# Dasch0/nenbody

Hardware: AMD Instinct MI355X
Metric: body-updates/sec (N x steps/s) at N=131072, all-pairs gravity + Euler step (higher is better)
Workload: dtype f32

## Files before the change

include/nenbody.h:

```cpp
#ifndef NENBODY_H
#define NENBODY_H

#include <stddef.h>
#include <stdint.h>

#ifdef __cplusplus
extern "C" {
#endif

#define NB_ABI_VERSION 2

typedef enum nb_status {
    NB_OK = 0,
    NB_ERR_INVALID = -1,
    NB_ERR_NO_DEVICE = -2,
    NB_ERR_HIP = -3,
    NB_ERR_ALLOC = -4,
    NB_ERR_STATE = -5,
    NB_ERR_UNSUPPORTED = -6
} nb_status;

typedef enum nb_mode {
    NB_MODE_STRICT = 0,
    NB_MODE_FAST = 1
// ... 86 lines not shown

int nb_scenes_create(uint32_t scenes, uint32_t n, const nb_params *params, nb_scenes **out);
void nb_scenes_destroy(nb_scenes *ctx);
int nb_scenes_upload(nb_scenes *ctx, const float *pos_xyz, const float *vel_xyz);
int nb_scenes_step(nb_scenes *ctx, uint32_t k);
int nb_scenes_step_boids(nb_scenes *ctx, uint32_t k, const nb_boids_params *params);
int nb_scenes_download(nb_scenes *ctx, float *pos_xyz, float *vel_xyz, float *inst_16);
int nb_scenes_device_state(nb_scenes *ctx, const void **pos_rec, const void **vel_rec, const void **inst_16);
int nb_scenes_sync(nb_scenes *ctx);
uint64_t nb_scenes_steps(const nb_scenes *ctx);
const char *nb_scenes_last_error(const nb_scenes *ctx);


#include "nenbody_scenes_seen.h"


#include "nenbody_scenes_located.h"

#define NB_FRAME_MAX_DIM 4096u
int nb_camera_at(nb_ctx *ctx, const float *eye_xyz, const float *dir_xyz, const float *up_xyz, const float *cp16, float *out16);
int nb_frame(nb_ctx *ctx, const float *cam16, uint32_t width, uint32_t height, uint32_t flags, uint32_t *ids, float *depth, float *rgba,
             uint32_t *bgra8);

#define NB_FRAME_MSAA_MAX_DIM 2048u
int nb_frame_sample_offsets(float *out16);
int nb_frame_msaa(nb_ctx *ctx, const float *cam16, uint32_t width, uint32_t height, uint32_t flags, uint32_t *ids8, float *depth8,
                  float *rgba, uint32_t *bgra8);

int nb_download(nb_ctx *ctx, float *pos_xyz, float *vel_xyz, float *inst_16n);

int nb_sync(nb_ctx *ctx);

uint64_t nb_steps_done(const nb_ctx *ctx);

int nb_update_instance_nbody(float *instances_16n, size_t n_instances, float *positions_xyz, size_t n_positions,
                             float *old_positions_xyz, size_t n_old_positions, float *velocities_xyz, size_t n_velocities,
                             float *old_velocities_xyz, size_t n_old_velocities, const nb_params *params);
int nb_update_instance_boids(float *instances_16n, size_t n_instances, float *positions_xyz, size_t n_positions,
                             float *old_positions_xyz, size_t n_old_positions, float *velocities_xyz, size_t n_velocities,
                             float *old_velocities_xyz, size_t n_old_velocities, const nb_boids_params *params);
int nb_update_instance_random(float *instances_16n, size_t n_instances, float *positions_xyz, size_t n_positions,
                              float *velocities_xyz, size_t n_velocities);
int nb_update_instance_random_seeded(float *instances_16n, size_t n_instances, float *positions_xyz, size_t n_positions,
                                     float *velocities_xyz, size_t n_velocities, uint64_t seed, uint64_t step);
void nb_update_random_seed(uint64_t seed);

void nb_update_release(void);


size_t nb_scratch_bytes(const nb_params *params, uint32_t n_total, uint32_t count);

int nb_launch_step(const nb_params *params, uint32_t n_total, uint32_t first, uint32_t count, const void *pos_in,
                   void *pos_out, void *vel, void *scratch, size_t scratch_bytes, void *stream);

enum { NB_PHASE_RANGE = 0, NB_PHASE_REST = 1 };
size_t nb_scratch_bytes_phased(const nb_params *params, uint32_t n_total, uint32_t count, uint32_t j_lo, uint32_t j_hi);
int nb_launch_step_phase(const nb_params *params, uint32_t n_total, uint32_t first, uint32_t count, uint32_t j_lo, uint32_t j_hi,
                         int phase, const void *pos_in, void *pos_out, void *vel, void *scratch, size_t scratch_bytes, void *stream);

int nb_ring_partners(const nb_params *params, uint32_t n_total, uint32_t first, uint32_t count);
size_t nb_ring_scratch_bytes(const nb_params *params, uint32_t n_total, uint32_t first, uint32_t count);
int nb_launch_ring_fold(const nb_params *params, uint32_t n_total, uint32_t first, uint32_t count, const void *pos_in, void *sums,
                        void *scratch, size_t scratch_bytes, void *stream);
int nb_launch_ring_finish(const nb_params *params, uint32_t n_total, uint32_t first, uint32_t count, const void *pos_in, void *pos_out,
                          void *vel, const void *sums, const void *recv, void *stream);

enum { NB_RING_OWN = 1, NB_RING_REST = 2, NB_RING_SUMS = 3, NB_RING_OWN_READY = 4 };
int nb_ring_phased(const nb_params *params, uint32_t n_total, uint32_t first, uint32_t count);
int nb_launch_ring_fold_phase(const nb_params *params, uint32_t n_total, uint32_t first, uint32_t count, int phase, const void *pos_in,
                              void *sums, void *scratch, size_t scratch_bytes, void *stream);
int nb_launch_ring_finish_phase(const nb_params *params, uint32_t n_total, uint32_t first, uint32_t count, const void *pos_in, void *pos_out,
                                void *vel, const void *sums, const void *recv, void *scratch, size_t scratch_bytes, void *stream);

int nb_launch_boids_step(const nb_boids_params *params, uint32_t n_total, uint32_t first, uint32_t count, const void *pos_in,
                         const void *vel_in, void *pos_out, void *vel_out, void *stream);

size_t nb_boids_split_scratch_bytes(const nb_boids_params *params, uint32_t n_total, uint32_t count);
int nb_launch_boids_step_split(const nb_boids_params *params, uint32_t n_total, uint32_t first, uint32_t count, const void *pos_in,
                               const void *vel_in, void *pos_out, void *vel_out, void *scratch, size_t scratch_bytes, void *stream);

int nb_launch_instances(uint32_t count, const void *pos, const void *vel, void *inst_16n, void *stream);

int nb_launch_cameras(uint32_t count, const void *eyes, const void *dirs, const float *up_xyz, const float *cp16, void *out_16n,
                      void *stream);

int nb_launch_eyes(uint32_t n_total, uint32_t first, uint32_t count, const void *cams_16, const void *inst_16n, uint32_t width,
                   uint32_t flags, void *ids, void *depth, void *stream);

int nb_launch_seen(uint32_t count, uint32_t width, const void *ids_rows, const void *depth_rows, void *seen_count, void *seen_ids,
                   void *seen_depth, void *seen_cols, void *stream);

int nb_launch_boids_seen_step(const nb_boids_params *params, uint32_t n_total, uint32_t first, uint32_t count, const void *pos_in,
                              const void *vel_in, const void *seen_count, const void *seen_ids, uint32_t stride, void *pos_out,
                              void *vel_out, void *stream);

int nb_seen_located_launch(uint32_t count, uint32_t width, const void *ids_rows, const void *depth_rows, const void *seen_count,
                           const void *seen_ids, const void *seen_depth, const void *eyes, const void *dirs, const float *up_xyz,
                           const float *cp16, void *seen_col, void *seen_rel, void *stream);

int nb_nbody_located_step_launch(const nb_params *params, uint32_t n_total, uint32_t first, uint32_t count, const void *pos_in,
                                 const void *vel_in, const void *seen_count, const void *seen_rel, uint32_t stride, void *pos_out,
                                 void *vel_out, void *stream);

int nb_launch_eyes_colour(uint32_t n_total, uint32_t first, uint32_t count, const void *cams_16, const void *inst_16n, uint32_t width,
                          uint32_t flags, const void *skin, uint32_t tw, uint32_t th, void *ids, void *depth, void *rgba, void *bgra8,
                          void *stream);
// ... 72 lines not shown
```

include/nenbody_diag.h:

```cpp
#ifndef NENBODY_DIAG_H
#define NENBODY_DIAG_H

#include "nenbody.h"

#ifdef __cplusplus
extern "C" {
#endif

int nb_selftest_divide(const nb_params *params, uint64_t pairs, uint64_t seed, uint64_t *mismatches, float *bad_pair);

int nb_selftest_ladder(uint32_t first_significand, uint32_t count, uint64_t *mismatches, float *bad_pair);
int nb_selftest_rcp_scaling(int k_lo, int k_hi, uint64_t *violations);

int nb_selftest_matrices(uint32_t count, uint64_t seed, uint64_t *mismatches, float *bad_velocity);
int nb_selftest_libm(int fn, uint32_t first, uint64_t count, uint32_t x_bits, uint64_t *mismatches, uint32_t *first_bad);

int nb_selftest_valu_rate(int mix, double seconds, double *lane_ops_per_s, double *clock_mhz);

int nb_diag_step_clock(const nb_params *params, uint32_t n, double seconds, double *clock_mhz, double *wave_cycles,
                       double *kernel_ms);

int nb_diag_enable_env(int on);
int nb_debug_reload_env(void);

int nb_diag_rccl_solo(int on);

int nb_diag_legacy_forms(void);

int nb_diag_peers_lossy(int on);

int nb_diag_plan(const nb_params *params, uint32_t n_total, uint32_t count, char *out, size_t out_bytes);

#ifdef __cplusplus
}
#endif
#endif
```

nenbody_amd/_lib.py:

```python
from __future__ import annotations

import ctypes
import os
from ctypes import POINTER, c_char_p, c_float, c_int, c_size_t, c_uint32, c_uint64, c_void_p

_HERE = os.path.dirname(os.path.abspath(__file__))
LIB_PATH = os.environ.get("NENBODY_LIB") or os.path.join(_HERE, "lib", "libnenbody_hip.so")

NB_ABI_VERSION = 2
NB_OK = 0
NB_ERR_INVALID = -1
NB_ERR_NO_DEVICE = -2
NB_ERR_HIP = -3
NB_ERR_ALLOC = -4
NB_ERR_STATE = -5
NB_ERR_UNSUPPORTED = -6

NB_MODE_STRICT = 0
NB_MODE_FAST = 1
NB_PHASE_RANGE = 0
NB_PHASE_REST = 1
NB_RING_OWN, NB_RING_REST, NB_RING_SUMS, NB_RING_OWN_READY = 1, 2, 3, 4
NB_SCENES_MAX_BODIES = 2048
NB_EYES_NONE = 0xFFFFFFFF
NB_EYES_SEE_SELF = 1
NB_EYES_MAX_WIDTH = 4096
NB_EYES_MAX_SKIN = 2048
NB_EYES_SAMPLES = 8
NB_EYES_MSAA_MAX_WIDTH = 2048
NB_FRAME_MAX_DIM = 4096
NB_FRAME_MSAA_MAX_DIM = 2048

_STATUS_NAMES = {
    NB_ERR_INVALID: "NB_ERR_INVALID",
    NB_ERR_NO_DEVICE: "NB_ERR_NO_DEVICE",
    NB_ERR_HIP: "NB_ERR_HIP",
    NB_ERR_ALLOC: "NB_ERR_ALLOC",
    NB_ERR_STATE: "NB_ERR_STATE",
    NB_ERR_UNSUPPORTED: "NB_ERR_UNSUPPORTED",
}


class NbParams(ctypes.Structure):

    _fields_ = [("dt", c_float), ("G", c_float), ("bias", c_float), ("tile", c_uint32), ("mode", c_uint32)]

    def __repr__(self) -> str:
        return f"NbParams(dt={self.dt}, G={self.G}, bias={self.bias}, tile={self.tile}, mode={self.mode})"


class NbBoidsParams(ctypes.Structure):

    _fields_ = [("dt", c_float), ("rule_1_distance", c_float), ("rule_2_distance", c_float), ("rule_3_distance", c_float),
                ("rule_1_scale", c_float), ("rule_2_scale", c_float), ("rule_3_scale", c_float), ("tile", c_uint32)]


class NbError(RuntimeError):

    def __init__(self, status: int, message: str):
        self.status = status
        super().__init__(f"{_STATUS_NAMES.get(status, status)}: {message}")


NB_COMM_ID_BYTES = 128
GATHER_FN = ctypes.CFUNCTYPE(c_int, c_void_p, c_void_p, c_size_t, c_int, c_int, c_void_p)

RING_FN = ctypes.CFUNCTYPE(c_int, c_void_p, c_void_p, c_void_p, c_size_t, c_int, c_int, c_int, c_void_p)

PROTOTYPES = {
    "nb_abi_version": (c_int, []),
    "nb_default_params": (None, [POINTER(NbParams)]),
    "nb_device_count": (c_int, []),
    "nb_last_error": (c_char_p, [c_void_p]),
    "nb_init_state": (c_int, [c_uint64, c_uint32, c_void_p, c_void_p]),
# ... 28 lines not shown
    "nb_launch_seen": (c_int, [c_uint32, c_uint32, c_void_p, c_void_p, c_void_p, c_void_p, c_void_p, c_void_p, c_void_p]),
    "nb_step_boids_seen": (c_int, [c_void_p, c_uint32, POINTER(NbBoidsParams), c_void_p, c_void_p, c_uint32, c_uint32]),
    "nb_launch_boids_seen_step": (
        c_int, [POINTER(NbBoidsParams), c_uint32, c_uint32, c_uint32, c_void_p, c_void_p, c_void_p, c_void_p, c_uint32, c_void_p, c_void_p,
                c_void_p]),
    "nb_eyes_located": (
        c_int, [c_void_p, c_uint32, c_uint32, c_void_p, c_void_p, c_uint32, c_uint32, c_void_p, c_void_p, c_void_p, c_void_p, c_void_p,
                c_void_p]),
    "nb_seen_located_launch": (
        c_int, [c_uint32, c_uint32, c_void_p, c_void_p, c_void_p, c_void_p, c_void_p, c_void_p, c_void_p, c_void_p, c_void_p, c_void_p,
                c_void_p, c_void_p]),
    "nb_step_nbody_located": (c_int, [c_void_p, c_uint32, c_void_p, c_void_p, c_uint32, c_uint32]),
    "nb_nbody_located_step_launch": (
        c_int, [POINTER(NbParams), c_uint32, c_uint32, c_uint32, c_void_p, c_void_p, c_void_p, c_void_p, c_uint32, c_void_p, c_void_p,
                c_void_p]),
    "nb_scenes_nbody_step_launch": (c_int, [POINTER(NbParams), c_uint32, c_uint32, c_uint32, c_void_p, c_void_p, c_void_p]),
    "nb_scenes_boids_step_launch": (c_int, [POINTER(NbBoidsParams), c_uint32, c_uint32, c_uint32, c_void_p, c_void_p, c_void_p]),
    "nb_scenes_create": (c_int, [c_uint32, c_uint32, POINTER(NbParams), POINTER(c_void_p)]),
    "nb_scenes_destroy": (None, [c_void_p]),
    "nb_scenes_upload": (c_int, [c_void_p, c_void_p, c_void_p]),
    "nb_scenes_step": (c_int, [c_void_p, c_uint32]),
    "nb_scenes_step_boids": (c_int, [c_void_p, c_uint32, POINTER(NbBoidsParams)]),
    "nb_scenes_download": (c_int, [c_void_p, c_void_p, c_void_p, c_void_p]),
    "nb_scenes_device_state": (c_int, [c_void_p, POINTER(c_void_p), POINTER(c_void_p), POINTER(c_void_p)]),
    "nb_scenes_sync": (c_int, [c_void_p]),
    "nb_scenes_steps": (c_uint64, [c_void_p]),
    "nb_scenes_last_error": (c_char_p, [c_void_p]),
    "nb_srgb_decode_table": (c_int, [c_void_p]),
    "nb_srgb_encode": (c_int, [c_void_p, c_size_t, c_void_p]),
    "nb_camera_at": (c_int, [c_void_p, c_void_p, c_void_p, c_void_p, c_void_p, c_void_p]),
    "nb_frame": (c_int, [c_void_p, c_void_p, c_uint32, c_uint32, c_uint32, c_void_p, c_void_p, c_void_p, c_void_p]),
    "nb_frame_scratch_bytes": (c_size_t, [c_uint32, c_uint32]),
    "nb_launch_frame": (c_int, [c_uint32, c_void_p, c_void_p, c_uint32, c_uint32, c_uint32, c_void_p, c_uint32, c_uint32, c_void_p,
                                c_void_p, c_void_p, c_void_p, c_void_p, c_void_p]),
    "nb_frame_sample_offsets": (c_int, [c_void_p]),
    "nb_frame_msaa": (c_int, [c_void_p, c_void_p, c_uint32, c_uint32, c_uint32, c_void_p, c_void_p, c_void_p, c_void_p]),
    "nb_frame_msaa_scratch_bytes": (c_size_t, [c_uint32, c_uint32]),
    "nb_launch_frame_msaa": (c_int, [c_uint32, c_void_p, c_void_p, c_uint32, c_uint32, c_uint32, c_void_p, c_uint32, c_uint32, c_void_p,
                                     c_void_p, c_void_p, c_void_p, c_void_p, c_void_p]),
    "nb_launch_random_step": (c_int, [c_uint32, c_uint32, c_void_p, c_void_p, c_uint64, c_uint64, c_void_p]),
    "nb_update_instance_nbody": (c_int, [c_void_p, c_size_t] * 5 + [POINTER(NbParams)]),
    "nb_update_instance_boids": (c_int, [c_void_p, c_size_t] * 5 + [POINTER(NbBoidsParams)]),
    "nb_update_instance_random": (c_int, [c_void_p, c_size_t, c_void_p, c_size_t, c_void_p, c_size_t]),
    "nb_update_instance_random_seeded": (c_int, [c_void_p, c_size_t, c_void_p, c_size_t, c_void_p, c_size_t, c_uint64, c_uint64]),
    "nb_update_random_seed": (None, [c_uint64]),
    "nb_update_release": (None, []),
    "nb_sync": (c_int, [c_void_p]),
    "nb_steps_done": (c_uint64, [c_void_p]),
    "nb_scratch_bytes": (c_size_t, [POINTER(NbParams), c_uint32, c_uint32]),
    "nb_launch_step": (
        c_int,
        [POINTER(NbParams), c_uint32, c_uint32, c_uint32, c_void_p, c_void_p, c_void_p, c_void_p, c_size_t, c_void_p],
    ),
    "nb_scratch_bytes_phased": (c_size_t, [POINTER(NbParams), c_uint32, c_uint32, c_uint32, c_uint32]),
    "nb_launch_step_phase": (
        c_int,
        [POINTER(NbParams), c_uint32, c_uint32, c_uint32, c_uint32, c_uint32, c_int, c_void_p, c_void_p, c_void_p, c_void_p, c_size_t,
         c_void_p],
    ),
    "nb_ring_partners": (c_int, [POINTER(NbParams), c_uint32, c_uint32, c_uint32]),
    "nb_ring_scratch_bytes": (c_size_t, [POINTER(NbParams), c_uint32, c_uint32, c_uint32]),
    "nb_launch_ring_fold": (c_int, [POINTER(NbParams), c_uint32, c_uint32, c_uint32, c_void_p, c_void_p, c_void_p, c_size_t, c_void_p]),
    "nb_ring_phased": (c_int, [POINTER(NbParams), c_uint32, c_uint32, c_uint32]),
    "nb_launch_ring_fold_phase": (c_int, [POINTER(NbParams), c_uint32, c_uint32, c_uint32, c_int, c_void_p, c_void_p, c_void_p, c_size_t, c_void_p]),
    "nb_launch_ring_finish": (
        c_int, [POINTER(NbParams), c_uint32, c_uint32, c_uint32, c_void_p, c_void_p, c_void_p, c_void_p, c_void_p, c_void_p]),
    "nb_launch_ring_finish_phase": (
        c_int, [POINTER(NbParams), c_uint32, c_uint32, c_uint32, c_void_p, c_void_p, c_void_p, c_void_p, c_void_p, c_void_p, c_size_t, c_void_p]),
    "nb_launch_status": (c_int, [c_void_p]),
    "nb_launch_instances": (c_int, [c_uint32, c_void_p, c_void_p, c_void_p, c_void_p]),
    "nb_launch_pack": (c_int, [c_uint32, c_void_p, c_void_p, c_void_p]),
    "nb_launch_unpack": (c_int, [c_uint32, c_void_p, c_void_p, c_void_p]),
    "nb_comm_id": (c_int, [c_void_p]),
    "nb_shard_create": (c_int, [c_uint32, c_int, c_int, POINTER(NbParams), POINTER(c_void_p)]),
    "nb_shard_destroy": (None, [c_void_p]),
    "nb_shard_use_rccl": (c_int, [c_void_p, c_void_p]),
    "nb_shard_use_gather": (c_int, [c_void_p, GATHER_FN, c_void_p]),
    "nb_shard_set_overlap": (c_int, [c_void_p, c_int]),
    "nb_shard_use_ring": (c_int, [c_void_p, RING_FN, c_void_p]),
    "nb_shard_set_pairs": (c_int, [c_void_p, c_int]),
    "nb_shard_pairs_partners": (c_int, [c_void_p]),
    "nb_shard_pairs_overlapped": (c_int, [c_void_p]),
    "nb_shard_verify_exchanges": (c_int, [c_void_p, POINTER(c_int), POINTER(c_int)]),
    "nb_shard_peer_export": (c_int, [c_void_p, c_void_p]),
    "nb_shard_peer_import": (c_int, [c_void_p, c_void_p]),
    "nb_shard_use_peers": (c_int, [c_void_p, c_int]),
    "nb_peers_blob_bytes": (c_size_t, []),
    "nb_peers_create": (c_int, [c_int, c_int, POINTER(c_void_p)]),
    "nb_peers_destroy": (None, [c_void_p]),
    "nb_peers_last_error": (c_char_p, [c_void_p]),
    "nb_peers_export": (c_int, [c_void_p, POINTER(c_void_p), POINTER(c_size_t), c_int, c_void_p]),
    "nb_peers_import": (c_int, [c_void_p, c_void_p]),
    "nb_peers_probe": (c_int, [c_void_p, c_uint32]),
    "nb_peers_signal": (c_int, [c_void_p, c_int, c_void_p]),
    "nb_peers_gather": (c_int, [c_void_p, c_int, c_int, c_size_t, c_void_p]),
    "nb_peers_ring": (c_int, [c_void_p, c_int, c_int, c_void_p, c_size_t, c_int, c_void_p]),
    "nb_shard_choose_form": (c_int, [c_void_p, c_uint32, POINTER(c_int), POINTER(ctypes.c_double)]),
    "nb_shard_set_boids_split": (c_int, [c_void_p, c_int]),
    "nb_shard_range": (c_int, [c_void_p, POINTER(c_uint32), POINTER(c_uint32)]),
    "nb_shard_upload": (c_int, [c_void_p, c_void_p, c_void_p]),
    "nb_shard_step": (c_int, [c_void_p, c_uint32]),
    "nb_shard_step_boids": (c_int, [c_void_p, c_uint32, POINTER(NbBoidsParams)]),
    "nb_shard_download": (c_int, [c_void_p, c_void_p, c_void_p, c_void_p]),
    "nb_shard_sync": (c_int, [c_void_p]),
    "nb_shard_last_error": (c_char_p, [c_void_p]),
}

SCENES_SEEN_PROTOTYPES = {
    "nb_scenes_boids_seen_step_launch": (c_int, [POINTER(NbBoidsParams), c_uint32, c_uint32, c_void_p, c_void_p, c_uint32, c_void_p, c_void_p,
                                                 c_void_p, c_void_p, c_void_p]),
    "nb_scenes_seen_launch": (c_int, [c_uint32, c_uint32, c_uint32, c_uint32, c_void_p, c_void_p, c_uint32, c_void_p, c_void_p, c_void_p]),
    "nb_scenes_step_boids_seen": (c_int, [c_void_p, c_uint32, POINTER(NbBoidsParams), c_void_p, c_void_p, c_uint32]),
    "nb_scenes_eyes_seen": (c_int, [c_void_p, c_uint32, c_uint32, c_void_p, c_void_p, c_uint32, c_void_p, c_void_p]),
}

SCENES_LOCATED_PROTOTYPES = {
    "nb_scenes_nbody_located_step_launch": (c_int, [POINTER(NbParams), c_uint32, c_uint32, c_void_p, c_void_p, c_void_p, c_void_p, c_uint32,
                                                    c_void_p, c_void_p, c_void_p, c_void_p, c_void_p]),
    "nb_scenes_located_launch": (c_int, [c_uint32, c_uint32, c_uint32, c_uint32, c_void_p, c_void_p, c_void_p, c_void_p, c_void_p, c_uint32,
                                         c_void_p, c_void_p, c_void_p, c_void_p, c_void_p, c_void_p]),
    "nb_scenes_step_nbody_located": (c_int, [c_void_p, c_uint32, c_void_p, c_void_p, c_uint32]),
    "nb_scenes_eyes_located": (c_int, [c_void_p, c_uint32, c_uint32, c_void_p, c_void_p, c_uint32, c_void_p, c_void_p, c_void_p, c_void_p,
                                       c_void_p]),
}

DIAG_PROTOTYPES = {
    "nb_selftest_ladder": (c_int, [c_uint32, c_uint32, POINTER(c_uint64), c_void_p]),
    "nb_selftest_rcp_scaling": (c_int, [c_int, c_int, POINTER(c_uint64)]),
    "nb_selftest_matrices": (c_int, [c_uint32, c_uint64, POINTER(c_uint64), c_void_p]),
    "nb_selftest_libm": (c_int, [c_int, c_uint32, c_uint64, c_uint32, POINTER(c_uint64), POINTER(c_uint32)]),
    "nb_selftest_divide": (c_int, [POINTER(NbParams), c_uint64, c_uint64, POINTER(c_uint64), c_void_p]),
    "nb_selftest_valu_rate": (c_int, [c_int, ctypes.c_double, POINTER(ctypes.c_double), POINTER(ctypes.c_double)]),
    "nb_diag_step_clock": (c_int, [POINTER(NbParams), c_uint32, ctypes.c_double, POINTER(ctypes.c_double), POINTER(ctypes.c_double),
                                   POINTER(ctypes.c_double)]),
    "nb_debug_reload_env": (c_int, []),
    "nb_diag_enable_env": (c_int, [c_int]),
    "nb_diag_rccl_solo": (c_int, [c_int]),
    "nb_diag_legacy_forms": (c_int, []),
    "nb_diag_peers_lossy": (c_int, [c_int]),
    "nb_diag_plan": (c_int, [POINTER(NbParams), c_uint32, c_uint32, ctypes.c_char_p, c_size_t]),
}

_lib = None


def _preload_torch_hip_runtime() -> None:
    if os.environ.get("NENBODY_SYSTEM_HIP"):
        return
    try:
        import importlib.util

        spec = importlib.util.find_spec("torch")
        if spec is None or not spec.submodule_search_locations:
            return
        path = os.path.join(list(spec.submodule_search_locations)[0], "lib", "libamdhip64.so")
        if os.path.exists(path):
            ctypes.CDLL(path, mode=ctypes.RTLD_GLOBAL)
            rccl = os.path.join(os.path.dirname(path), "librccl.so")
            if os.path.exists(rccl):
                os.environ.setdefault("NENBODY_RCCL", rccl)
    except Exception:
        pass


_loaded = {}


def _bind(path: str) -> ctypes.CDLL:
    if path in _loaded:
        return _loaded[path]
    if not os.path.exists(path):
        raise ImportError(
            f"{path} is missing: build it with `make -C nenbody_amd/csrc` (hipcc, gfx950). "
            "nenbody_amd has no CPU fallback."
        )
    _preload_torch_hip_runtime()
    lib = ctypes.CDLL(path)
    for name, (restype, argtypes) in list(PROTOTYPES.items()) + list(SCENES_SEEN_PROTOTYPES.items()) + list(SCENES_LOCATED_PROTOTYPES.items()) \
            + list(DIAG_PROTOTYPES.items()):
        fn = getattr(lib, name)
        fn.restype = restype
        fn.argtypes = argtypes
    got = lib.nb_abi_version()
    if got != NB_ABI_VERSION:
        raise ImportError(f"{os.path.basename(path)} ABI {got} != binding ABI {NB_ABI_VERSION}")
    _loaded[path] = lib
    return lib


def load() -> ctypes.CDLL:
    global _lib
    if _lib is None:
        _lib = _bind(LIB_PATH)
# ... 92 lines not shown
```

nenbody_amd/csrc/nb_api.hip:

```cpp
#include <hip/hip_runtime.h>
#include <dlfcn.h>

#include <cmath>
#include <cstdlib>
#include <algorithm>
#include <atomic>
#include <chrono>
#include <cstring>
#include <mutex>
#include <new>
#include <string>
#include <thread>
#include <vector>

#include "../../include/nenbody.h"
#include "../../include/nenbody_diag.h"
#include "nb_kernels.h"
#include "nb_plan.h"
#include "nb_eyes.h"
#include "nb_frame.h"
#include "nb_seen.h"
#include "nb_located.h"
#include "nb_scenes.h"
#define NB_SRGB_TABLE static const
// ... 17 lines not shown
using nbp::valid_tile;

Knob read_knob(const char *name)
{
    Knob k;
    const char *s = std::getenv(name);
    if (s && *s) {
        k.set = true;
        k.v = (uint32_t)std::strtoul(s, nullptr, 10);
    }
    return k;
}

std::atomic<const DebugOverrides *> g_overrides{nullptr};
std::atomic<bool> g_env_enabled{false};
std::atomic<bool> g_rccl_solo{false};
std::mutex g_overrides_mu;

const DebugOverrides *parse_overrides(uint32_t generation)
{
    DebugOverrides *d = new DebugOverrides();
    d->generation = generation;
    d->roctx = read_knob("NB_ROCTX");
    if (!g_env_enabled.load(std::memory_order_relaxed)) return d;
    for (const nbp::KnobName &k : nbp::kKnobNames) d->*k.knob = read_knob(k.name);
    return d;
}

const DebugOverrides &overrides()
{
    const DebugOverrides *d = g_overrides.load(std::memory_order_acquire);
    if (d) return *d;
    std::lock_guard<std::mutex> lock(g_overrides_mu);
    d = g_overrides.load(std::memory_order_acquire);
    if (!d) {
        d = parse_overrides(1);
        g_overrides.store(d, std::memory_order_release);
    }
    return *d;
}

int make_plan(const nb_params &p, uint32_t n_total, uint32_t count, Plan *out, std::string *err)
{
    return nbp::make_plan(p, n_total, count, overrides(), out, err);
}

struct KernelSizes {
    size_t planes_bytes(uint32_t n) const { return nbk::strict_bc_scratch_bytes(n); }
    uint32_t pairs_chunk(uint32_t n, uint32_t chunk) const { return nbk::fast_pairs_chunk(n, chunk); }
    uint32_t pairs_rows(uint32_t n, uint32_t w, uint32_t np) const { return nbk::fast_pairs_rows(n, w, np); }
    size_t pairs_scratch_floats(uint32_t n, uint32_t w, uint32_t np, uint32_t chunk) const { return nbk::fast_pairs_scratch_floats(n, w, np, chunk); }
};
size_t plan_scratch_bytes(const Plan &pl, uint32_t count) { return nbp::plan_scratch_bytes(pl, count, KernelSizes{}); }

struct PlanKey {
    nb_params p;
    uint32_t shape[4];
    uint32_t generation;
};
PlanKey plan_key(const nb_params &p, uint32_t s0, uint32_t s1, uint32_t s2 = 0, uint32_t s3 = 0)
{
    PlanKey k;
    std::memset(&k, 0, sizeof(k));
    k.p = p;
    k.shape[0] = s0;
    k.shape[1] = s1;
    k.shape[2] = s2;
    k.shape[3] = s3;
    k.generation = overrides().generation;
    return k;
}
template <typename Key, typename Value, int N>
class PlanCache {
    struct Entry {
        bool valid = false;
        Key key;
        Value value;
    };
    Entry entries_[N];
    int next_ = 0;

public:
    template <typename Make>
    int get(const Key &key, const Value **out, Make make)
    {
        for (const Entry &e : entries_)
            if (e.valid && std::memcmp(&e.key, &key, sizeof(Key)) == 0) {
                *out = &e.value;
                return NB_OK;
            }
        Value v;
        int rc = make(&v);
        if (rc != NB_OK) return rc;
        Entry &e = entries_[next_];
        next_ = (next_ + 1) % N;
        e.valid = true;
        e.key = key;
        e.value = v;
        *out = &e.value;
        return NB_OK;
    }
};

int cached_plan(const nb_params &p, uint32_t n_total, uint32_t count, const Plan **out, std::string *err)
{
    thread_local PlanCache<PlanKey, Plan, 4> cache;
// ... 91 lines not shown
}

struct StatusWord {
    uint32_t *w = nullptr;
    bool dirty = false;
};

int status_word_for_launch(StatusWord *sw, std::string *err)
{
    if (!sw->w) {
        hipError_t e = hipMalloc((void **)&sw->w, 64);
        if (e == hipSuccess) e = hipMemset(sw->w, 0, 64);
        if (e != hipSuccess) {
            *err = std::string("nb: allocating the status word failed: ") + hipGetErrorString(e);
            return e == hipErrorOutOfMemory ? NB_ERR_ALLOC : NB_ERR_HIP;
        }
    }
    sw->dirty = true;
    return NB_OK;
}

int check_status(StatusWord *sw, std::string *err)
{
    if (!sw->dirty) return NB_OK;
    sw->dirty = false;
    return check_status_word(sw->w, err);
}

nbk::StepArgs step_args(const nb_params &p, const Plan &pl, uint32_t n_total, uint32_t first, uint32_t count, const void *pos_in,
                        void *pos_out, void *vel, void *partial = nullptr)
{
    nbk::StepArgs a{};
    a.pos_in = (const float4 *)pos_in;
    a.pos_out = (float4 *)pos_out;
    a.vel = (float4 *)vel;
    a.partial = (float4 *)partial;
    a.n_total = n_total;
    a.first = first;
    a.count = count;
    a.dt = p.dt;
    a.G = p.G;
    a.bias = p.bias;
    a.j_count = n_total;
    a.hole_lo = 0xffffffffu;
    nbp::plan_step_args(pl, &a);
    return a;
}

struct Launchers {
    const nbk::StepArgs &a;
    void *scratch;
    uint32_t *status;
    hipStream_t s;
    hipError_t strict(uint32_t tile, uint32_t unroll, uint32_t lanes) const { return nbk::launch_strict(a, tile, unroll, lanes, s); }
    hipError_t strict_pc(uint32_t producers) const { return nbk::launch_strict_pc(a, producers, s); }
    hipError_t strict_bc() const { return nbk::launch_strict_bc(a, scratch, status, s); }
    hipError_t strict_sl(uint32_t shape) const { return nbk::launch_strict_sl(a, shape, scratch, s); }
    hipError_t fast(uint32_t tile, uint32_t ib, uint32_t groups, uint32_t slices) const { return nbk::launch_fast(a, tile, ib, groups, slices, s); }
    hipError_t fast_wave(uint32_t tile, uint32_t ib, uint32_t waves, uint32_t slices) const { return nbk::launch_fast_wave(a, tile, ib, waves, slices, s); }
    hipError_t fast_sl(uint32_t ib, uint32_t slices) const { return nbk::launch_fast_sl(a, ib, slices, scratch, s); }
    hipError_t fast_pairs(uint32_t w, uint32_t np, uint32_t chunk) const { return nbk::launch_fast_pairs(a, w, np, chunk, scratch, s); }
};
hipError_t launch_planned(const Plan &pl, const nbk::StepArgs &a, void *scratch, uint32_t *status, hipStream_t stream)
{
    return nbp::visit_launch(pl, Launchers{a, scratch, status, stream});
}

int launch_status(hipError_t e, const char *what, std::string *err)
{
    if (e == hipSuccess) return NB_OK;
    *err = std::string(what) + hipGetErrorString(e);
    return NB_ERR_HIP;
}

int launch_step_planned(const nb_params &p, const Plan &pl, uint32_t n_total, uint32_t first, uint32_t count,
                        const void *pos_in, void *pos_out, void *vel, void *scratch, hipStream_t stream, std::string *err,
                        StatusWord *sw = nullptr)
{
    const nbk::StepArgs a = step_args(p, pl, n_total, first, count, pos_in, pos_out, vel, scratch);
    uint32_t *status = nullptr;
    if (nbp::form_info(pl.form).status_word) {
        int rc = sw ? status_word_for_launch(sw, err) : device_status_word(&status, err);
        if (rc != NB_OK) return rc;
        if (sw) status = sw->w;
    }
    hipError_t e = launch_planned(pl, a, scratch, status, stream);
    if (e == hipErrorNotSupported) {
        *err = "nb: this launch shape is one of the legacy forms (NB_STRICT_PC / NB_STRICT_LANES / NB_STRICT_UNROLL / NB_STRICT_SL=2,3 / "
               "NB_FAST_WAVES / NB_FAST_GROUPS / NB_FAST_PAIRS_W): this library was built without them (make -C nenbody_amd/csrc legacy "
               "builds libnenbody_hip_legacy.so, which holds every form)";
        return NB_ERR_UNSUPPORTED;
    }
    return launch_status(e, "nb: kernel launch failed: ", err);
}

int check_device(std::string *err)
{
    static std::atomic<bool> seen{false};
    if (seen.load(std::memory_order_relaxed)) return NB_OK;
    int n = 0;
    hipError_t e = hipGetDeviceCount(&n);
    if (e != hipSuccess || n <= 0) {
        (void)hipGetLastError();
        *err = std::string("nb: no HIP device available (") + (e == hipSuccess ? "0 devices" : hipGetErrorString(e)) +
               "); this library has no CPU path";
        return NB_ERR_NO_DEVICE;
    }
    seen.store(true, std::memory_order_relaxed);
    return NB_OK;
}

float sqrt_threshold(float r)
{
    if (!(r > 0.0f)) return -1.0f;
    uint32_t lo = 0u, hi = 0x7f7fffffu;
    auto below = [&](uint32_t b) {
        float x;
        std::memcpy(&x, &b, 4);
        return std::sqrt(x) < r;
    };
    if (!below(lo)) return -1.0f;
    if (below(hi)) {
        float x;
        std::memcpy(&x, &hi, 4);
        return x;
    }
    while (hi - lo > 1u) {
        const uint32_t mid = lo + (hi - lo) / 2u;
        if (below(mid))
            lo = mid;
        else
            hi = mid;
    }
    float x;
    std::memcpy(&x, &lo, 4);
    return x;
}

float rule3_always_bound(float t3)
// ... 196 lines not shown
        p = nullptr;
        cells = 0;
    }
    hipError_t reserve(size_t want)
    {
        if (want <= cells) return hipSuccess;
        release();
        const hipError_t e = hipMalloc((void **)&p, want * sizeof(T));
        if (e == hipSuccess)
            cells = want;
        else
            p = nullptr;
        return e;
    }
    void swap(DeviceBuffer &other)
    {
        std::swap(p, other.p);
        std::swap(cells, other.cells);
    }
};

struct nb_ctx {
    uint32_t n = 0;
    nb_params p{};
    Plan plan{};
    hipStream_t stream = nullptr;
    DeviceBuffer<float4> pos[2];
    DeviceBuffer<float4> vel;
    DeviceBuffer<float4> vel_alt;
    DeviceBuffer<float> stage;
    DeviceBuffer<float4> inst;
    DeviceBuffer<float4> cams;
    DeviceBuffer<uint32_t> eye_ids;
    DeviceBuffer<float> eye_depth;
    DeviceBuffer<float4> eye_rgba;
    DeviceBuffer<uint32_t> eye_bgra;
    DeviceBuffer<uint32_t> seen_count;
    DeviceBuffer<uint32_t> seen_ids;
    DeviceBuffer<float> seen_depth;
    DeviceBuffer<uint32_t> seen_cols;
    DeviceBuffer<uint32_t> loc_col;
    DeviceBuffer<float4> loc_rel;
    DeviceBuffer<float> skin;
    uint32_t skin_w = 0, skin_h = 0;
    DeviceBuffer<uint64_t> frame_keys;
    DeviceBuffer<float4> frame_cam;
    DeviceBuffer<float> xfer;
    float *hxfer = nullptr;
    float *hxfer_dev = nullptr;
    DeviceBuffer<uint32_t> done_counter;
    uint32_t done_seq = 0, polled_calls = 0;
    uint32_t poll_holdoff = 0, poll_backoff = 0;
    DeviceBuffer<char> scratch;
    StatusWord status;
    int cur = 0;
    bool uploaded = false;
    uint64_t steps = 0;
    std::string err;
    ~nb_ctx()
    {
        if (hxfer) (void)hipHostFree(hxfer);
        if (status.w) (void)hipFree(status.w);
    }
};

#define NB_HIP(ctx, call)                                                                          \
    do {                                                                                           \
        hipError_t e_ = (call);                                                                    \
        if (e_ != hipSuccess) {                                                                    \
            (ctx)->err = std::string("nb: " #call " failed: ") + hipGetErrorString(e_);            \
            return (e_ == hipErrorOutOfMemory) ? NB_ERR_ALLOC : NB_ERR_HIP;                        \
        }                                                                                          \
    } while (0)

static const char kCallUpload[] = " (call nb_upload first)";
static const char kCallScenesUpload[] = " (call nb_scenes_upload first)";
template <typename Ctx>
static int ctx_check(Ctx *ctx, const char *fn, const char *state_hint = nullptr)
{
    if (!ctx) {
        g_tls_error = std::string(fn) + ": ctx is null";
        return NB_ERR_INVALID;
    }
    if (state_hint && !ctx->uploaded) {
        ctx->err = std::string(fn) + ": no state uploaded" + state_hint;
        return NB_ERR_STATE;
    }
    return NB_OK;
}

static hipError_t launch_matrices(uint32_t n, const float4 *pos, const float4 *vel, DeviceBuffer<float4> *inst, hipStream_t stream)
{
    const hipError_t e = inst->reserve((size_t)n * 4);
    if (e != hipSuccess) return e;
    return nbk::launch_instances(n, pos, vel, inst->p, stream, overrides().inst_device_libm.on() ? 1u : 0u);
}

static void step_done(nb_ctx *c, bool wrote_vel_alt)
{
    c->cur ^= 1;
    if (wrote_vel_alt) c->vel.swap(c->vel_alt);
    c->steps++;
}

NB_EXPORT int nb_abi_version(void) { return NB_ABI_VERSION; }

NB_EXPORT void nb_default_params(nb_params *p)
{
    if (!p) return;
    p->dt = 0.1f;
    p->G = 0.001f;
    p->bias = 0.0000001f;
    p->tile = 0;
    p->mode = NB_MODE_STRICT;
}

NB_EXPORT int nb_device_count(void)
{
    int n = 0;
    hipError_t e = hipGetDeviceCount(&n);
    if (e != hipSuccess) {
        (void)hipGetLastError();
        g_tls_error = std::string("nb: hipGetDeviceCount failed: ") + hipGetErrorString(e);
        return NB_ERR_NO_DEVICE;
    }
    return n;
}

NB_EXPORT const char *nb_last_error(const nb_ctx *ctx) { return ctx ? ctx->err.c_str() : g_tls_error.c_str(); }

NB_EXPORT int nb_init_state(uint64_t seed, uint32_t n, float *pos_xyz, float *vel_xyz)
{
    if (!pos_xyz || !vel_xyz) {
        g_tls_error = "nb_init_state: null array";
        return NB_ERR_INVALID;
    }
    uint64_t s = seed;
    for (uint32_t i = 0; i < n; ++i) {
        vel_xyz[3 * (size_t)i + 0] = uniform_f32(s, -0.0f, 0.1f);
        vel_xyz[3 * (size_t)i + 1] = uniform_f32(s, -0.0f, 0.1f);
        vel_xyz[3 * (size_t)i + 2] = 0.0f;
    }
    for (uint32_t i = 0; i < n; ++i) {
        pos_xyz[3 * (size_t)i + 0] = uniform_f32(s, -100.0f, 100.0f);
        pos_xyz[3 * (size_t)i + 1] = uniform_f32(s, -100.0f, 100.0f);
        pos_xyz[3 * (size_t)i + 2] = 0.0f;
    }
    return NB_OK;
}

NB_EXPORT void nb_destroy(nb_ctx *ctx)
{
// ... 49 lines not shown
    }
    if (polled) {
        d.counter = c->done_counter.p;
        d.word = (uint32_t *)(c->hxfer_dev + 22 * (size_t)c->n + kDoneWordAt);
        d.seq = ++c->done_seq ? c->done_seq : ++c->done_seq;
    }
    return d;
}

static inline void cpu_relax()
{
#if defined(__x86_64__) || defined(__i386__)
    __builtin_ia32_pause();
#elif defined(__aarch64__)
    __asm__ __volatile__("yield");
#else
    std::this_thread::yield();
#endif
}

static int wait_export(nb_ctx *c, const nbk::ExportDone &d)
{
    if (d.word) {
        const volatile uint32_t *const w = (const volatile uint32_t *)(c->hxfer + 22 * (size_t)c->n + kDoneWordAt);
        const auto kPollBudget = std::chrono::microseconds(overrides().dropin_poll_budget_us.or_else(2000u));
        const auto t0 = std::chrono::steady_clock::now();
        for (uint32_t spins = 1;; ++spins) {
            if (*w == d.seq) {
                std::atomic_thread_fence(std::memory_order_acquire);
                c->poll_backoff = 0;
                if ((++c->polled_calls & 1023u) == 0u) NB_HIP(c, hipStreamSynchronize(c->stream));
                return NB_OK;
            }
            if ((spins & 255u) == 0u && std::chrono::steady_clock::now() - t0 > kPollBudget) break;
            cpu_relax();
        }
        c->poll_backoff = c->poll_backoff ? std::min(c->poll_backoff * 2u, 4096u) : 64u;
        c->poll_holdoff = c->poll_backoff;
        NB_HIP(c, hipStreamSynchronize(c->stream));
        if (*w != d.seq) NB_HIP(c, hipMemsetAsync(c->done_counter.p, 0, sizeof(uint32_t), c->stream));
        return NB_OK;
    }
    NB_HIP(c, hipStreamSynchronize(c->stream));
    return NB_OK;
}

static int create_impl(nb_ctx *c)
{
    NB_HIP(c, hipStreamCreateWithFlags(&c->stream, hipStreamNonBlocking));
    NB_HIP(c, c->pos[0].reserve(c->n));
    NB_HIP(c, c->pos[1].reserve(c->n));
    NB_HIP(c, c->vel.reserve(c->n));
    NB_HIP(c, c->stage.reserve((size_t)c->n * 3));
    NB_HIP(c, c->scratch.reserve(plan_scratch_bytes(c->plan, c->n)));
    return NB_OK;
}

NB_EXPORT int nb_create(uint32_t n, uint32_t n_devices, const nb_params *params, nb_ctx **out)
{
    if (!out) {
        g_tls_error = "nb_create: out is null";
        return NB_ERR_INVALID;
    }
    *out = nullptr;
    if (n_devices != 1) {
        g_tls_error =
            "nb_create: n_devices must be 1 (one process drives one GPU; shard with nb_launch_step and an all-gather)";
        return NB_ERR_UNSUPPORTED;
    }
    const nb_params p = params_or_default(params);
    Plan plan;
    int rc = make_plan(p, n, n, &plan, &g_tls_error);
    if (rc != NB_OK) return rc;
    rc = check_device(&g_tls_error);
    if (rc != NB_OK) return rc;
    nb_ctx *c = new (std::nothrow) nb_ctx();
    if (!c) {
        g_tls_error = "nb_create: out of host memory";
        return NB_ERR_ALLOC;
    }
    c->n = n;
    c->p = p;
    c->plan = plan;
    rc = create_impl(c);
    if (rc != NB_OK) {
        g_tls_error = c->err;
        nb_destroy(c);
        return rc;
    }
    *out = c;
    return NB_OK;
}


static int small_import(nb_ctx *c, const float *pos_xyz, const float *vel_xyz)
{
    const size_t n = c->n, bytes = n * 3 * sizeof(float);
    std::memcpy(c->hxfer, pos_xyz, bytes);
    std::memcpy(c->hxfer + 3 * n, vel_xyz, bytes);
    float *src = c->hxfer_dev;
    if (!small_set_zero_copy(c->n)) {
        NB_HIP(c, hipMemcpyAsync(c->xfer.p, c->hxfer, 2 * bytes, hipMemcpyHostToDevice, c->stream));
        src = c->xfer.p;
    }
    NB_HIP(c, nbk::launch_import(c->n, src, src + 3 * n, c->pos[0].p, c->vel.p, c->stream));
    return NB_OK;
}

static int small_export(nb_ctx *c, bool inst, bool pos, bool vel, bool *with_status)
{
    const size_t n = c->n;
    const bool zero_copy = small_set_zero_copy(c->n);
    float *const dst = zero_copy ? c->hxfer_dev : c->xfer.p;
    const bool ws = *with_status = c->status.dirty && c->status.w;
    const nbk::ExportDone done = export_done(c, small_set_poll(c->n));
    NB_HIP(c, nbk::launch_export(c->n, c->pos[c->cur].p, c->vel.p, inst ? (float4 *)dst : nullptr, pos ? dst + 16 * n : nullptr,
                                 vel ? dst + 19 * n : nullptr, ws ? c->status.w : nullptr, ws ? (uint32_t *)(dst + 22 * n) : nullptr,
                                 c->stream, overrides().inst_device_libm.on() ? 1u : 0u, done));
    if (!zero_copy) {
        const size_t lo = inst ? 0 : (pos ? 16 * n : 19 * n), hi = ws ? 22 * n + 1 : vel ? 22 * n : (pos ? 19 * n : 16 * n);
        NB_HIP(c, hipMemcpyAsync(c->hxfer + lo, c->xfer.p + lo, (hi - lo) * sizeof(float), hipMemcpyDeviceToHost, c->stream));
    }
    return wait_export(c, done);
}

NB_EXPORT int nb_upload(nb_ctx *ctx, const float *pos_xyz, const float *vel_xyz)
{
    int rc = ctx_check(ctx, "nb_upload");
    if (rc != NB_OK) return rc;
    if (!pos_xyz || !vel_xyz) {
        ctx->err = "nb_upload: null array";
        return NB_ERR_INVALID;
    }
    const size_t bytes = (size_t)ctx->n * 3 * sizeof(float);
    ctx->cur = 0;
    if (ctx->n <= kRoundtripMax) {
        rc = ensure_xfer(ctx);
        if (rc != NB_OK) return rc;
        NB_HIP(ctx, hipStreamSynchronize(ctx->stream));
        rc = small_import(ctx, pos_xyz, vel_xyz);
        if (rc != NB_OK) return rc;
        NB_HIP(ctx, hipStreamSynchronize(ctx->stream));
        ctx->uploaded = true;
        ctx->steps = 0;
        return NB_OK;
    }
    NB_HIP(ctx, hipMemcpyAsync(ctx->stage.p, pos_xyz, bytes, hipMemcpyHostToDevice, ctx->stream));
    NB_HIP(ctx, nbk::launch_pack(ctx->n, ctx->stage.p, ctx->pos[0].p, ctx->stream));
    NB_HIP(ctx, hipStreamSynchronize(ctx->stream));
    NB_HIP(ctx, hipMemcpyAsync(ctx->stage.p, vel_xyz, bytes, hipMemcpyHostToDevice, ctx->stream));
    NB_HIP(ctx, nbk::launch_pack(ctx->n, ctx->stage.p, ctx->vel.p, ctx->stream));
    NB_HIP(ctx, hipStreamSynchronize(ctx->stream));
    ctx->uploaded = true;
    ctx->steps = 0;
    return NB_OK;
}

NB_EXPORT int nb_step(nb_ctx *ctx, uint32_t k)
{
    int rc = ctx_check(ctx, "nb_step", kCallUpload);
    if (rc != NB_OK) return rc;
    RoctxRange range("nb_step");
    for (uint32_t s = 0; s < k; ++s) {
        rc = launch_step_planned(ctx->p, ctx->plan, ctx->n, 0, ctx->n, ctx->pos[ctx->cur].p, ctx->pos[ctx->cur ^ 1].p, ctx->vel.p,
                                 ctx->scratch.p, ctx->stream, &ctx->err, &ctx->status);
        if (rc != NB_OK) return rc;
        step_done(ctx, false);
    }
    return NB_OK;
}

NB_EXPORT void nb_boids_default_params(nb_boids_params *p)
{
    if (!p) return;
    p->dt = 0.04f;
    p->rule_1_distance = 1000.0f;
    p->rule_2_distance = 5.0f;
    p->rule_3_distance = 500.0f;
    p->rule_1_scale = 0.02f;
    p->rule_2_scale = 0.05f;
    p->rule_3_scale = 0.5f;
    p->tile = 0;
}

NB_EXPORT int nb_step_boids(nb_ctx *ctx, uint32_t k, const nb_boids_params *params)
{
    int rc = ctx_check(ctx, "nb_step_boids", kCallUpload);
    if (rc != NB_OK) return rc;
    const nb_boids_params p = boids_params_or_default(params);
    nbk::BoidsArgs a;
    uint32_t tile = 0;
    rc = make_boids_args(p, ctx->n, 0, ctx->n, &a, &tile, &ctx->err);
    if (rc != NB_OK) return rc;
    NB_HIP(ctx, ctx->vel_alt.reserve(ctx->n));
    RoctxRange range("nb_step_boids");
    for (uint32_t s = 0; s < k; ++s) {
        a.pos_in = ctx->pos[ctx->cur].p;
        a.pos_out = ctx->pos[ctx->cur ^ 1].p;
        a.vel_in = ctx->vel.p;
        a.vel_out = ctx->vel_alt.p;
        NB_HIP(ctx, nbk::launch_boids(a, tile, boids_form(a.count), ctx->stream));
        step_done(ctx, true);
    }
    return NB_OK;
}

NB_EXPORT int nb_step_random(nb_ctx *ctx, uint32_t k, uint64_t seed)
{
    const int rc = ctx_check(ctx, "nb_step_random", kCallUpload);
    if (rc != NB_OK) return rc;
    for (uint32_t s = 0; s < k; ++s) {
        NB_HIP(ctx, nbk::launch_random(0, ctx->n, ctx->pos[ctx->cur].p, ctx->vel.p, seed, ctx->steps, ctx->stream));
        ctx->steps++;
    }
    return NB_OK;
}

NB_EXPORT int nb_device_state(nb_ctx *ctx, const void **pos_rec, const void **vel_rec, const void **inst_16n)
{
    const int rc = ctx_check(ctx, "nb_device_state", "");
    if (rc != NB_OK) return rc;
    if (inst_16n) {
        NB_HIP(ctx, launch_matrices(ctx->n, ctx->pos[ctx->cur].p, ctx->vel.p, &ctx->inst, ctx->stream));
        *inst_16n = ctx->inst.p;
    }
    if (pos_rec) *pos_rec = ctx->pos[ctx->cur].p;
    if (vel_rec) *vel_rec = ctx->vel.p;
    return NB_OK;
}

NB_EXPORT int nb_camera_constant(float vertical_fov_deg, float aspect_ratio, float near_plane, float far_plane, float *cp16)
{
    if (!cp16) {
        g_tls_error = "nb_camera_constant: cp16 is null";
        return NB_ERR_INVALID;
    }
    const float pi = (float)3.14159265358979323846;
    const float fovy = vertical_fov_deg * (float)(3.14159265358979323846 / 180.0);
    if (!(fovy > 0.0f) || !(fovy < pi) || !(aspect_ratio != 0.0f) || !(near_plane > 0.0f) || !(far_plane > 0.0f) || !(far_plane != near_plane)) {
        g_tls_error = "nb_camera_constant: cgmath::perspective asserts 0 < fovy < 180 degrees, aspect != 0, near > 0, far > 0, far != near";
        return NB_ERR_INVALID;
    }
    const float f = 1.0f / std::tan(fovy / 2.0f);
    float proj[16] = {0.0f};
    proj[0] = f / aspect_ratio;
    proj[5] = f;
    proj[10] = (far_plane + near_plane) / (near_plane - far_plane);
    proj[11] = -1.0f;
    proj[14] = ((2.0f * far_plane) * near_plane) / (near_plane - far_plane);
    const float corr[16] = {1.0f, 0.0f, 0.0f, 0.0f, 0.0f, 1.0f, 0.0f, 0.0f, 0.0f, 0.0f, 0.5f, 0.0f, 0.0f, 0.0f, 0.5f, 1.0f};
    for (int col = 0; col < 4; ++col)
        for (int row = 0; row < 4; ++row) {
            const float t0 = corr[row] * proj[4 * col], t1 = corr[4 + row] * proj[4 * col + 1];
            const float t2 = corr[8 + row] * proj[4 * col + 2], t3 = corr[12 + row] * proj[4 * col + 3];
            cp16[4 * col + row] = ((t0 + t1) + t2) + t3;
        }
    return NB_OK;
}

NB_EXPORT int nb_cameras(nb_ctx *ctx, const float *up_xyz, const float *cp16, float *out_16n)
{
    int rc = ctx_check(ctx, "nb_cameras");
    if (rc != NB_OK) return rc;
    if (!up_xyz || !cp16 || !out_16n) {
// ... 359 lines not shown
NB_EXPORT uint64_t nb_steps_done(const nb_ctx *ctx) { return ctx ? ctx->steps : 0; }

NB_EXPORT int nb_download(nb_ctx *ctx, float *pos_xyz, float *vel_xyz, float *inst_16n)
{
    int rc = ctx_check(ctx, "nb_download", "");
    if (rc != NB_OK) return rc;
    const size_t bytes = (size_t)ctx->n * 3 * sizeof(float);
    if (ctx->n <= kRoundtripMax && (pos_xyz || vel_xyz || inst_16n)) {
        rc = ensure_xfer(ctx);
        if (rc != NB_OK) return rc;
        const size_t n = ctx->n;
        bool with_status = false;
        rc = small_export(ctx, inst_16n != nullptr, pos_xyz != nullptr, vel_xyz != nullptr, &with_status);
        if (rc != NB_OK) return rc;
        if (inst_16n) std::memcpy(inst_16n, ctx->hxfer, n * 16 * sizeof(float));
        if (pos_xyz) std::memcpy(pos_xyz, ctx->hxfer + 16 * n, bytes);
        if (vel_xyz) std::memcpy(vel_xyz, ctx->hxfer + 19 * n, bytes);
        return status_from_tail(ctx, with_status);
    }
    if (pos_xyz) {
        NB_HIP(ctx, nbk::launch_unpack(ctx->n, ctx->pos[ctx->cur].p, ctx->stage.p, ctx->stream));
        NB_HIP(ctx, hipMemcpyAsync(pos_xyz, ctx->stage.p, bytes, hipMemcpyDeviceToHost, ctx->stream));
        NB_HIP(ctx, hipStreamSynchronize(ctx->stream));
    }
    if (vel_xyz) {
        NB_HIP(ctx, nbk::launch_unpack(ctx->n, ctx->vel.p, ctx->stage.p, ctx->stream));
        NB_HIP(ctx, hipMemcpyAsync(vel_xyz, ctx->stage.p, bytes, hipMemcpyDeviceToHost, ctx->stream));
        NB_HIP(ctx, hipStreamSynchronize(ctx->stream));
    }
    if (inst_16n) {
        NB_HIP(ctx, launch_matrices(ctx->n, ctx->pos[ctx->cur].p, ctx->vel.p, &ctx->inst, ctx->stream));
        NB_HIP(ctx, hipMemcpyAsync(inst_16n, ctx->inst.p, (size_t)ctx->n * 16 * sizeof(float), hipMemcpyDeviceToHost,
                                   ctx->stream));
        NB_HIP(ctx, hipStreamSynchronize(ctx->stream));
    }
    if (!pos_xyz && !vel_xyz && !inst_16n) NB_HIP(ctx, hipStreamSynchronize(ctx->stream));
    return check_status(&ctx->status, &ctx->err);
}

#include "nb_dropin.inc"

#include "nb_selftest.inc"


NB_EXPORT size_t nb_scratch_bytes(const nb_params *params, uint32_t n_total, uint32_t count)
{
    const nb_params p = params_or_default(params);
    Plan pl;
    std::string err;
    if (make_plan(p, n_total, count, &pl, &err) != NB_OK) return 0;
    return plan_scratch_bytes(pl, count);
}

NB_EXPORT int nb_launch_step(const nb_params *params, uint32_t n_total, uint32_t first, uint32_t count, const void *pos_in,
                             void *pos_out, void *vel, void *scratch, size_t scratch_bytes, void *stream)
{
    const nb_params p = params_or_default(params);
    if (!pos_in || !pos_out || !vel || pos_in == pos_out) {
        g_tls_error = "nb_launch_step: pos_in, pos_out, vel must be non-null and pos_out must not alias pos_in";
        return NB_ERR_INVALID;
    }
    if ((uint64_t)first + (uint64_t)count > (uint64_t)n_total) {
        g_tls_error = "nb_launch_step: [first, first+count) exceeds n_total";
        return NB_ERR_INVALID;
    }
    const Plan *pl = nullptr;
    int rc = cached_plan(p, n_total, count, &pl, &g_tls_error);
    if (rc != NB_OK) return rc;
    const size_t need = plan_scratch_bytes(*pl, count);
    if (need && (!scratch || scratch_bytes < need)) {
        g_tls_error = "nb_launch_step: scratch smaller than nb_scratch_bytes()";
        return NB_ERR_INVALID;
    }
    rc = device_for_launch(pos_in, stream, SelectDevice::kForNullStream);
    if (rc != NB_OK) return rc;
    return launch_step_planned(p, *pl, n_total, first, count, pos_in, pos_out, vel, scratch, (hipStream_t)stream, &g_tls_error);
}

NB_EXPORT int nb_launch_status(void *stream)
{
    int rc = check_device(&g_tls_error);
    if (rc != NB_OK) return rc;
    int cur = -1, restore = -1;
    if (stream) {
        hipDevice_t sdev = -1;
        if (hipStreamGetDevice((hipStream_t)stream, &sdev) == hipSuccess && hipGetDevice(&cur) == hipSuccess && sdev >= 0 && sdev != cur) {
            if (hipSetDevice(sdev) == hipSuccess) restore = cur;
        } else {
            (void)hipGetLastError();
        }
    }
    hipError_t e = hipStreamSynchronize((hipStream_t)stream);
    if (e != hipSuccess) {
        g_tls_error = std::string("nb_launch_status: hipStreamSynchronize failed: ") + hipGetErrorString(e);
        rc = NB_ERR_HIP;
    } else {
        rc = check_device_status(&g_tls_error);
    }
    if (restore >= 0) (void)hipSetDevice(restore);
    return rc;
}

namespace {
int make_phase_plan(const nb_params &p, uint32_t n_total, uint32_t count, uint32_t j_lo, uint32_t j_hi, PhasePlan *out, std::string *err)
{
    return nbp::make_phase_plan(p, n_total, count, j_lo, j_hi, overrides(), out, err);
}
size_t phase_scratch_bytes(const PhasePlan &pp, uint32_t count) { return nbp::phase_scratch_bytes(pp, count, KernelSizes{}); }

int cached_phase_plan(const nb_params &p, uint32_t n_total, uint32_t count, uint32_t j_lo, uint32_t j_hi, const PhasePlan **out,
                      std::string *err)
{
    thread_local PlanCache<PlanKey, PhasePlan, 2> cache;
    return cache.get(plan_key(p, n_total, count, j_lo, j_hi), out,
                     [&](PhasePlan *pp) { return make_phase_plan(p, n_total, count, j_lo, j_hi, pp, err); });
}
}

NB_EXPORT size_t nb_scratch_bytes_phased(const nb_params *params, uint32_t n_total, uint32_t count, uint32_t j_lo, uint32_t j_hi)
{
    const nb_params p = params_or_default(params);
    PhasePlan pp;
    std::string err;
    if (make_phase_plan(p, n_total, count, j_lo, j_hi, &pp, &err) != NB_OK) return 0;
    return phase_scratch_bytes(pp, count);
}

namespace {
int launch_phase_planned(const nb_params &p, const PhasePlan &pp, uint32_t n_total, uint32_t first, uint32_t count, uint32_t j_lo,
// ... 23 lines not shown
        a.hole_len = pp.len[0];
        e = fold(1, false, 0, 0);
        if (e == hipSuccess) e = nbk::launch_integrate_partials(a, pp.slices[0] + pp.slices[1], stream);
    }
    return launch_status(e, "nb: kernel launch failed (step phase): ", err);
}
}

NB_EXPORT int nb_launch_step_phase(const nb_params *params, uint32_t n_total, uint32_t first, uint32_t count, uint32_t j_lo,
                                   uint32_t j_hi, int phase, const void *pos_in, void *pos_out, void *vel, void *scratch,
                                   size_t scratch_bytes, void *stream)
{
    const nb_params p = params_or_default(params);
    if (!pos_in || !pos_out || !vel || pos_in == pos_out || !scratch || (phase != NB_PHASE_RANGE && phase != NB_PHASE_REST)) {
        g_tls_error = "nb_launch_step_phase: pos_in, pos_out, vel, scratch must be non-null, pos_out must not alias pos_in, phase is "
                      "NB_PHASE_RANGE or NB_PHASE_REST";
        return NB_ERR_INVALID;
    }
    if ((uint64_t)first + (uint64_t)count > (uint64_t)n_total) {
        g_tls_error = "nb_launch_step_phase: [first, first+count) exceeds n_total";
        return NB_ERR_INVALID;
    }
    const PhasePlan *ppp = nullptr;
    int rc = cached_phase_plan(p, n_total, count, j_lo, j_hi, &ppp, &g_tls_error);
    if (rc != NB_OK) return rc;
    const PhasePlan &pp = *ppp;
    if (scratch_bytes < phase_scratch_bytes(pp, count)) {
        g_tls_error = "nb_launch_step_phase: scratch smaller than nb_scratch_bytes_phased()";
        return NB_ERR_INVALID;
    }
    rc = device_for_launch(pos_in, stream, SelectDevice::kForNullStream);
    if (rc != NB_OK) return rc;
    return launch_phase_planned(p, pp, n_total, first, count, j_lo, phase, pos_in, pos_out, vel, scratch, (hipStream_t)stream, &g_tls_error);
}

#include "nb_ring_api.inc"


NB_EXPORT int nb_diag_legacy_forms(void)
{
#ifdef NB_LEGACY_FORMS
    return 1;
#else
    return 0;
#endif
}

NB_EXPORT int nb_diag_rccl_solo(int on)
{
    g_rccl_solo.store(on != 0, std::memory_order_relaxed);
    return NB_OK;
}

NB_EXPORT int nb_diag_plan(const nb_params *params, uint32_t n_total, uint32_t count, char *out, size_t out_bytes)
{
    if (!out || out_bytes == 0) {
        g_tls_error = "nb_diag_plan: out is null";
        return NB_ERR_INVALID;
    }
    const nb_params p = params_or_default(params);
    Plan pl;
    int rc = make_plan(p, n_total, count, &pl, &g_tls_error);
    if (rc != NB_OK) return rc;
    const std::string k = nbp::plan_kernels(pl, KernelSizes{});
    if (k.size() + 1 > out_bytes) {
        g_tls_error = "nb_diag_plan: out too small";
        return NB_ERR_INVALID;
    }
    std::memcpy(out, k.c_str(), k.size() + 1);
    return NB_OK;
}

namespace {
int reread_overrides(bool enable)
{
    std::lock_guard<std::mutex> lock(g_overrides_mu);
    g_env_enabled.store(enable, std::memory_order_relaxed);
    const DebugOverrides *old = g_overrides.load(std::memory_order_acquire);
    g_overrides.store(parse_overrides(old ? old->generation + 1u : 1u), std::memory_order_release);
    return NB_OK;
}
}
NB_EXPORT int nb_diag_enable_env(int on) { return reread_overrides(on != 0); }
NB_EXPORT int nb_debug_reload_env(void) { return reread_overrides(true); }

NB_EXPORT int nb_launch_boids_step(const nb_boids_params *params, uint32_t n_total, uint32_t first, uint32_t count,
                                   const void *pos_in, const void *vel_in, void *pos_out, void *vel_out, void *stream)
{
    const nb_boids_params p = boids_params_or_default(params);
    if (!pos_in || !vel_in || !pos_out || !vel_out || pos_in == pos_out || vel_in == vel_out) {
        g_tls_error = "nb_launch_boids_step: buffers must be non-null and the outputs must not alias the inputs";
        return NB_ERR_INVALID;
    }
    nbk::BoidsArgs a;
    uint32_t tile = 0;
    int rc = make_boids_args(p, n_total, first, count, &a, &tile, &g_tls_error);
    if (rc != NB_OK) return rc;
    rc = device_for_launch(pos_in, stream, SelectDevice::kAlways);
    if (rc != NB_OK) return rc;
    a.pos_in = (const float4 *)pos_in;
    a.vel_in = (const float4 *)vel_in;
    a.pos_out = (float4 *)pos_out;
    a.vel_out = (float4 *)vel_out;
    return launch_status(nbk::launch_boids(a, tile, boids_form(a.count), (hipStream_t)stream), "nb: boids kernel launch failed: ", &g_tls_error);
}

// ... 224 lines not shown
```

nenbody_amd/csrc/nb_kernels.h:

```cpp
#pragma once
#include <hip/hip_runtime.h>
#include <stdint.h>

namespace nbk {

struct StepArgs {
    const float4 *pos_in;
    float4 *pos_out;
    float4 *vel;
    float4 *partial;
    uint32_t n_total, first, count;
    float dt, G, bias;
    uint32_t lo_bits, hi_bits;
    uint32_t force_ieee;
    uint32_t force_3d;
    uint32_t j_chunk;
    uint32_t no_packed;
    uint32_t spin_budget;
    uint32_t bc_prio;
    uint32_t j_count, j_base, hole_lo, hole_len;
    uint32_t partial_row0;
    uint32_t always_partial;
    unsigned long long *stamps;
};

struct BoidsMaskK {
    float k1, tk1;
    float k2, tk2;
    float k3, tk3;
};

struct BoidsArgs {
    const float4 *pos_in;
    const float4 *vel_in;
    float4 *pos_out;
    float4 *vel_out;
    uint32_t n_total, first, count;
    float dt;
    float r1;
    float t2, t3;
    float s1, s2, s3;
    uint32_t force_flags;
    uint32_t vlim_bits;
    float4 *partial;
    uint32_t j_chunk;
    float4 *vtot;
    uint32_t *gflags;
    uint32_t mk_valid;
    BoidsMaskK mk;
};
hipError_t launch_boids(const BoidsArgs &a, uint32_t tile, uint32_t form, hipStream_t s);
hipError_t launch_boids_split(const BoidsArgs &a, uint32_t tile, uint32_t slices, hipStream_t s);

hipError_t launch_strict(const StepArgs &a, uint32_t tile, uint32_t unroll, uint32_t lanes, hipStream_t s);
hipError_t launch_strict_jp(const StepArgs &a, uint32_t tile, uint32_t unroll, uint32_t lanes, hipStream_t s);
hipError_t launch_strict_pc(const StepArgs &a, uint32_t producers, hipStream_t s);
hipError_t launch_strict_bc(const StepArgs &a, void *scratch, uint32_t *status, hipStream_t s);
size_t strict_bc_scratch_bytes(uint32_t n_total);
struct PlaneScratch {
    uint32_t *flags;
    float *px, *py, *pz;
    char *behind;
    uint32_t npad;
};
PlaneScratch plane_scratch(void *scratch, uint32_t n_total);
hipError_t launch_strict_sl(const StepArgs &a, uint32_t shape, void *scratch, hipStream_t s);
hipError_t launch_strict_sl_kernel(const StepArgs &a, uint32_t shape, const uint32_t *flags, uint32_t generation, const float *px,
                                   const float *py, const float *pz, hipStream_t s);
hipError_t launch_fast(const StepArgs &a, uint32_t tile, uint32_t ib, uint32_t groups, uint32_t slices, hipStream_t s);
hipError_t launch_fast_wave(const StepArgs &a, uint32_t tile, uint32_t ib, uint32_t waves, uint32_t slices, hipStream_t s);
hipError_t launch_fast_sl(const StepArgs &a, uint32_t ib, uint32_t slices, void *scratch, hipStream_t s);
hipError_t launch_fast_sl_phase(const StepArgs &a, uint32_t ib, uint32_t slices, bool range, uint32_t r0, uint32_t r1, void *scratch,
                                hipStream_t s);
hipError_t launch_fast_sl_kernel(const StepArgs &a, uint32_t ib, uint32_t slices, const uint32_t *flags, uint32_t generation,
                                 const float *px, const float *py, const float *pz, hipStream_t s);
hipError_t launch_fast_pairs(const StepArgs &a, uint32_t w, uint32_t np, uint32_t chunk, void *scratch, hipStream_t s);
hipError_t launch_fast_pairs_kernels(const StepArgs &a, uint32_t w, uint32_t np, uint32_t chunk, const uint32_t *flags, uint32_t generation,
                                     const float *px, const float *py, const float *pz, float *scratch, hipStream_t s);
uint32_t fast_pairs_rows(uint32_t n_total, uint32_t w, uint32_t np);
size_t fast_pairs_scratch_floats(uint32_t n_total, uint32_t w, uint32_t np, uint32_t chunk);
uint32_t fast_pairs_chunk(uint32_t n_total, uint32_t chunk);
uint32_t ring_partners(uint32_t n_total, uint32_t first, uint32_t count, uint32_t np);
size_t ring_scratch_floats(uint32_t n_total, uint32_t first, uint32_t count, uint32_t np, uint32_t ga, uint32_t wpb, uint32_t c4_own = 0, uint32_t c4_rest = 0,
                           uint32_t cap = 0);
bool ring_phased(uint32_t n_total, uint32_t first, uint32_t count, uint32_t np, uint32_t ga, uint32_t wpb, uint32_t *c4_own = nullptr, uint32_t *c4_rest = nullptr,
                 uint32_t *cap = nullptr);
hipError_t launch_fast_ring_phase(const StepArgs &a, uint32_t np, uint32_t ga, uint32_t wpb, uint32_t c4_own, uint32_t c4_rest, uint32_t cap, uint32_t what,
                                  void *scratch, float4 *sums, hipStream_t s);
hipError_t launch_ring_phase_kernels(const StepArgs &a, uint32_t np, uint32_t ga, uint32_t wpb, uint32_t c4_own, uint32_t c4_rest, uint32_t cap, uint32_t what,
                                     const uint32_t *flags, const float *px, const float *py, const float *pz, float *scratch, float4 *sums,
                                     hipStream_t s);
hipError_t launch_fast_ring(const StepArgs &a, uint32_t np, uint32_t ga, uint32_t wpb, void *scratch, float4 *sums, hipStream_t s);
hipError_t launch_fast_ring_kernels(const StepArgs &a, uint32_t np, uint32_t ga, uint32_t wpb, const uint32_t *flags, uint32_t generation,
                                    const float *px, const float *py, const float *pz, float *scratch, float4 *sums, hipStream_t s);
hipError_t launch_ring_finish(const StepArgs &a, const float4 *sums, const float4 *recv, uint32_t partners, hipStream_t s);
hipError_t launch_fast_ring_finish_phase(const StepArgs &a, uint32_t np, uint32_t ga, uint32_t wpb, uint32_t c4_own, uint32_t c4_rest, uint32_t cap, void *scratch,
                                         const float4 *sums, const float4 *recv, hipStream_t s);
hipError_t launch_ring_finish_phase_kernel(const StepArgs &a, uint32_t np, uint32_t ga, uint32_t wpb, uint32_t c4_own, uint32_t c4_rest, uint32_t cap,
                                           uint32_t *flags, float *px, float *py, float *pz, float *scratch, const float4 *sums, const float4 *recv,
                                           uint32_t gen_next, hipStream_t s);
hipError_t launch_integrate_partials(const StepArgs &a, uint32_t rows, hipStream_t s);
hipError_t launch_instances(uint32_t count, const float4 *pos, const float4 *vel, float4 *inst, hipStream_t s, uint32_t device_libm = 0);
hipError_t launch_cameras(uint32_t count, const float4 *eyes, const float4 *dirs, const float *up3, const float *cp16, float4 *out,
                          hipStream_t s);
hipError_t launch_random(uint32_t first, uint32_t count, float4 *pos, float4 *vel, uint64_t seed, uint64_t step, hipStream_t s);
hipError_t launch_divide_selftest(uint32_t blocks, uint64_t seed, uint32_t per_thread, int d_lo, int d_hi, int n_lo, int n_hi,
                                  unsigned long long *mismatches, float *first_bad, bool single_correction, hipStream_t s);
hipError_t launch_ladder_exhaustive(uint32_t first_md, uint32_t count_md, bool control, unsigned long long *mismatches, float *first_bad,
                                    hipStream_t s);
hipError_t launch_rcp_scaling(int k_lo, int k_hi, unsigned long long *violations, hipStream_t s);
hipError_t launch_libm_selftest(int fn, uint32_t first, uint32_t count, uint32_t other, uint32_t *out, hipStream_t s);
hipError_t launch_valu_stream(int mix, uint32_t blocks, uint32_t trips, float *sink, unsigned long long *stamps, hipStream_t s);
hipError_t launch_unstage(uint32_t slot, uint32_t world, const float4 *stage, float4 *pos, float4 *vel, hipStream_t s);
hipError_t launch_exchange_pattern(float4 *dst, uint32_t count, float rank, float salt, bool fill_nan, hipStream_t s);
hipError_t launch_exchange_check(const float4 *src, uint32_t count, float rank, float salt, uint32_t *mismatches, hipStream_t s);
constexpr int kPeerMax = 16;
struct PullArgs {
    const float4 *src[kPeerMax];
    float4 *dst[kPeerMax];
    uint32_t copies, records;
};
hipError_t launch_peer_pull(const PullArgs &a, hipStream_t s);
hipError_t launch_pack(uint32_t count, const float *xyz, float4 *rec, hipStream_t s);
hipError_t launch_unpack(uint32_t count, const float4 *rec, float *xyz, hipStream_t s);
hipError_t launch_import(uint32_t count, const float *pos_xyz, const float *vel_xyz, float4 *pos_rec, float4 *vel_rec, hipStream_t s);
struct ExportDone {
    uint32_t *counter = nullptr;
    uint32_t *word = nullptr;
    uint32_t seq = 0;
// ... 6 lines not shown
```

nenbody_amd/csrc/nb_launch.inc:

```

static inline uint32_t ceil_div(uint32_t a, uint32_t b) { return (a + b - 1u) / b; }

template <int TJ, int U, int S>
static hipError_t launch_strict_t(const StepArgs &a, hipStream_t s)
{
    hipLaunchKernelGGL((step_strict_kernel<TJ, U, S>), dim3(ceil_div(a.count, kBlock / S)), dim3(kBlock), 0, s, a);
    return hipGetLastError();
}

#define NBK_CASE(T, U_, S_) \
    if (tile == T && unroll == U_ && lanes == S_) return launch_strict_t<T, U_, S_>(a, s)

#ifdef NBK_NOSLP_TU
hipError_t launch_strict_jp(const StepArgs &a, uint32_t tile, uint32_t unroll, uint32_t lanes, hipStream_t s)
{
    NBK_CASE(256, 2, 16);
    NBK_CASE(1024, 2, 16);
#ifdef NB_LEGACY_FORMS
    NBK_CASE(256, 4, 2);
    NBK_CASE(256, 2, 2);
    NBK_CASE(256, 4, 4);
    NBK_CASE(256, 2, 4);
    NBK_CASE(256, 4, 8);
    NBK_CASE(256, 2, 8);
    NBK_CASE(256, 4, 16);
    NBK_CASE(1024, 4, 2);
    NBK_CASE(1024, 4, 4);
    NBK_CASE(1024, 4, 8);
    NBK_CASE(1024, 2, 8);
#endif
    return hipErrorNotSupported;
}

#else
hipError_t launch_strict_pc(const StepArgs &a, uint32_t producers, hipStream_t s)
{
#ifdef NB_LEGACY_FORMS
    if (producers == 8)
        hipLaunchKernelGGL(step_strict_pc_kernel<8>, dim3(ceil_div(a.count, 64)), dim3(PcShape<8>::kThreads), 0, s, a);
    else if (producers == 14)
        hipLaunchKernelGGL(step_strict_pc_kernel<14>, dim3(ceil_div(a.count, 64)), dim3(PcShape<14>::kThreads), 0, s, a);
    else
        return hipErrorInvalidValue;
    return hipGetLastError();
#else
    return hipErrorNotSupported;
#endif
}

constexpr size_t kPlaneSlackBytes = 64;
size_t strict_bc_scratch_bytes(uint32_t n_total) { return (size_t)kBcFlagsBytes + 3u * (size_t)bc_padded(n_total) * sizeof(float) + kPlaneSlackBytes; }

PlaneScratch plane_scratch(void *scratch, uint32_t n_total)
{
    PlaneScratch v;
    v.npad = bc_padded(n_total);
    v.flags = (uint32_t *)scratch;
    v.px = (float *)((char *)scratch + kBcFlagsBytes);
    v.py = v.px + v.npad;
    v.pz = v.py + v.npad;
    v.behind = (char *)scratch + strict_bc_scratch_bytes(n_total);
    return v;
}

static std::atomic<uint32_t> g_bc_generation{0};
static uint32_t next_plane_generation()
{
    uint32_t gen = g_bc_generation.fetch_add(1u, std::memory_order_relaxed) + 1u;
    if (gen == 0u) gen = g_bc_generation.fetch_add(1u, std::memory_order_relaxed) + 1u;
    return gen;
}

static void enqueue_planes(const StepArgs &a, const PlaneScratch &v, uint32_t lo_bits, uint32_t hi_bits, uint32_t gen, hipStream_t s)
{
    hipLaunchKernelGGL(planes_kernel, dim3(ceil_div(v.npad, kBlock)), dim3(kBlock), 0, s, a.n_total, v.npad, a.pos_in, v.px, v.py, v.pz,
                       v.flags, lo_bits, hi_bits, 0u, gen);
}
constexpr uint32_t kFastPlaneLoBits = 0u, kFastPlaneHiBits = 0x4d7fffffu;
static hipError_t launch_fast_planes(const StepArgs &a, const PlaneScratch &v, uint32_t gen, hipStream_t s)
{
    enqueue_planes(a, v, kFastPlaneLoBits, kFastPlaneHiBits, gen, s);
    return hipGetLastError();
}

hipError_t launch_strict_bc(const StepArgs &a, void *scratch, uint32_t *status, hipStream_t s)
{
    const PlaneScratch v = plane_scratch(scratch, a.n_total);
    const uint32_t gen = next_plane_generation();
    enqueue_planes(a, v, a.lo_bits, a.hi_bits, gen, s);
    hipLaunchKernelGGL(step_strict_bc_kernel, dim3(ceil_div(a.count, 64)), dim3(kBcThreads), 0, s, a, (const uint32_t *)v.flags, gen,
                       (const float *)v.px, (const float *)v.py, (const float *)v.pz, status);
    return hipGetLastError();
}

hipError_t launch_strict_sl(const StepArgs &a, uint32_t shape, void *scratch, hipStream_t s)
{
    const PlaneScratch v = plane_scratch(scratch, a.n_total);
    const uint32_t gen = next_plane_generation();
    enqueue_planes(a, v, a.lo_bits, a.hi_bits, gen, s);
    hipError_t e = hipGetLastError();
    if (e != hipSuccess) return e;
    return launch_strict_sl_kernel(a, shape, v.flags, gen, v.px, v.py, v.pz, s);
}

hipError_t launch_strict(const StepArgs &a, uint32_t tile, uint32_t unroll, uint32_t lanes, hipStream_t s)
{
    if (lanes > 1) return launch_strict_jp(a, tile, unroll, lanes, s);
    NBK_CASE(256, 8, 1);
    NBK_CASE(512, 8, 1);
    NBK_CASE(1024, 8, 1);
#ifdef NB_LEGACY_FORMS
    NBK_CASE(256, 4, 1);
    NBK_CASE(512, 4, 1);
    NBK_CASE(1024, 4, 1);
    NBK_CASE(1024, 16, 1);
#endif
    return hipErrorNotSupported;
}
#endif
#undef NBK_CASE

#ifndef NBK_NOSLP_TU
hipError_t launch_integrate_partials(const StepArgs &a, uint32_t rows, hipStream_t s)
{
    hipLaunchKernelGGL(integrate_partials_kernel, dim3(ceil_div(a.count, kBlock)), dim3(kBlock), 0, s, a, rows);
    return hipGetLastError();
}

template <int TJ, int IB, int G>
static hipError_t launch_fast_t(const StepArgs &a, uint32_t slices, hipStream_t s)
{
    hipLaunchKernelGGL((step_fast_kernel<TJ, IB, G>), dim3(ceil_div(a.count, kBlock * IB), slices), dim3(kBlock * G), 0, s, a);
    hipError_t e = hipGetLastError();
    if (e != hipSuccess || slices == 1 || a.always_partial) return e;
    return launch_integrate_partials(a, slices, s);
}

hipError_t launch_fast(const StepArgs &a, uint32_t tile, uint32_t ib, uint32_t groups, uint32_t slices, hipStream_t s)
{
#ifndef NB_LEGACY_FORMS
    return hipErrorNotSupported;
#else
#define NBK_CASE(T, I, G_) \
    if (tile == T && ib == I && groups == G_) return launch_fast_t<T, I, G_>(a, slices, s)
    NBK_CASE(256, 1, 1);
    NBK_CASE(256, 2, 1);
    NBK_CASE(256, 4, 1);
    NBK_CASE(512, 1, 1);
    NBK_CASE(512, 2, 1);
    NBK_CASE(512, 4, 1);
    NBK_CASE(1024, 1, 1);
    NBK_CASE(1024, 2, 1);
    NBK_CASE(1024, 4, 1);
    NBK_CASE(256, 1, 2);
    NBK_CASE(256, 2, 2);
    NBK_CASE(256, 4, 2);
    NBK_CASE(512, 1, 2);
    NBK_CASE(512, 2, 2);
    NBK_CASE(512, 4, 2);
    NBK_CASE(256, 1, 4);
    NBK_CASE(256, 2, 4);
    NBK_CASE(256, 4, 4);
    NBK_CASE(512, 1, 4);
    NBK_CASE(512, 2, 4);
    NBK_CASE(512, 4, 4);
#undef NBK_CASE
    return hipErrorInvalidValue;
#endif
}

template <int TJ, int IB, int W>
static hipError_t launch_fast_wave_t(const StepArgs &a, uint32_t slices, hipStream_t s)
{
    hipLaunchKernelGGL((step_fast_wave_kernel<TJ, IB, W>), dim3(ceil_div(a.count, 64 * IB), slices), dim3(64 * W), 0, s, a);
    hipError_t e = hipGetLastError();
    if (e != hipSuccess || slices == 1 || a.always_partial) return e;
    return launch_integrate_partials(a, slices, s);
}

hipError_t launch_fast_wave(const StepArgs &a, uint32_t tile, uint32_t ib, uint32_t waves, uint32_t slices, hipStream_t s)
{
#define NBK_CASE(T, I, W_) \
    if (tile == T && ib == I && waves == W_) return launch_fast_wave_t<T, I, W_>(a, slices, s)
    NBK_CASE(256, 1, 8);
    NBK_CASE(256, 2, 8);
    NBK_CASE(256, 4, 8);
    NBK_CASE(512, 2, 8);
    NBK_CASE(512, 4, 8);
#ifdef NB_LEGACY_FORMS
    NBK_CASE(256, 1, 1);
    NBK_CASE(256, 1, 4);
    NBK_CASE(256, 1, 16);
    NBK_CASE(256, 2, 1);
    NBK_CASE(256, 2, 4);
    NBK_CASE(256, 2, 16);
    NBK_CASE(256, 4, 1);
    NBK_CASE(256, 4, 4);
    NBK_CASE(256, 4, 16);
    NBK_CASE(512, 2, 4);
    NBK_CASE(512, 2, 16);
    NBK_CASE(512, 4, 4);
    NBK_CASE(512, 4, 16);
#endif
#undef NBK_CASE
    return hipErrorNotSupported;
}

hipError_t launch_fast_sl(const StepArgs &a_in, uint32_t ib, uint32_t slices, void *scratch, hipStream_t s)
{
    StepArgs a = a_in;
    const PlaneScratch v = plane_scratch(scratch, a.n_total);
    a.partial = (float4 *)v.behind;
    const uint32_t gen = next_plane_generation();
    hipError_t e = launch_fast_planes(a, v, gen, s);
    if (e != hipSuccess) return e;
    e = launch_fast_sl_kernel(a, ib, slices, v.flags, gen, v.px, v.py, v.pz, s);
    if (e != hipSuccess || slices == 1 || a.always_partial) return e;
    return launch_integrate_partials(a, slices, s);
}

hipError_t launch_fast_sl_phase(const StepArgs &a_in, uint32_t ib, uint32_t slices, bool range, uint32_t r0, uint32_t r1, void *scratch,
                                hipStream_t s)
{
    StepArgs a = a_in;
    const PlaneScratch v = plane_scratch(scratch, a.n_total);
    a.partial = (float4 *)v.behind;
    const uint32_t gen = next_plane_generation();
    hipError_t e;
    if (range) {
        hipLaunchKernelGGL(planes_range_kernel, dim3(ceil_div(a.n_total, kBlock)), dim3(kBlock), 0, s, a.n_total, a.pos_in, v.px, v.py, v.pz, v.flags,
                           r0, r1, a.first, a.first + a.count, kFastPlaneLoBits, kFastPlaneHiBits, 0u, gen);
        e = hipGetLastError();
    } else {
        e = launch_fast_planes(a, v, gen, s);
    }
    if (e != hipSuccess) return e;
    return launch_fast_sl_kernel(a, ib, slices, v.flags, gen, v.px, v.py, v.pz, s);
}

hipError_t launch_fast_pairs(const StepArgs &a, uint32_t w, uint32_t np, uint32_t chunk, void *scratch, hipStream_t s)
{
    const PlaneScratch v = plane_scratch(scratch, a.n_total);
    const uint32_t gen = next_plane_generation();
    hipError_t e = launch_fast_planes(a, v, gen, s);
    if (e != hipSuccess) return e;
    return launch_fast_pairs_kernels(a, w, np, chunk, v.flags, gen, v.px, v.py, v.pz, (float *)v.behind, s);
}

hipError_t launch_fast_ring(const StepArgs &a, uint32_t np, uint32_t ga, uint32_t wpb, void *scratch, float4 *sums, hipStream_t s)
{
    const PlaneScratch v = plane_scratch(scratch, a.n_total);
    const uint32_t gen = next_plane_generation();
    hipError_t e = launch_fast_planes(a, v, gen, s);
    if (e != hipSuccess) return e;
    return launch_fast_ring_kernels(a, np, ga, wpb, v.flags, gen, v.px, v.py, v.pz, (float *)v.behind, sums, s);
}

hipError_t launch_fast_ring_phase(const StepArgs &a, uint32_t np, uint32_t ga, uint32_t wpb, uint32_t c4_own, uint32_t c4_rest, uint32_t cap, uint32_t what,
                                  void *scratch, float4 *sums, hipStream_t s)
{
    const PlaneScratch v = plane_scratch(scratch, a.n_total);
    if (what == 1u || what == 2u) {
        const uint32_t gen = next_plane_generation();
        const bool own = what == 1u;
        const uint32_t r0 = own ? a.first : 0u, r1 = own ? a.first + a.count : a.n_total;
        hipLaunchKernelGGL(ring_planes_kernel, dim3(ceil_div(r1 - r0, kBlock)), dim3(kBlock), 0, s, a.n_total, a.pos_in, v.px, v.py, v.pz,
                           v.flags + (own ? kRingFlagsNext : kRingFlagsRest), r0, r1, gen, own ? (const uint32_t *)nullptr : v.flags + kRingFlagsNext,
                           own ? (uint32_t *)nullptr : v.flags + kRingFlagsOwn);
        hipError_t e = hipGetLastError();
        if (e != hipSuccess) return e;
    }
    return launch_ring_phase_kernels(a, np, ga, wpb, c4_own, c4_rest, cap, what, v.flags, v.px, v.py, v.pz, (float *)v.behind, sums, s);
}

hipError_t launch_fast_ring_finish_phase(const StepArgs &a, uint32_t np, uint32_t ga, uint32_t wpb, uint32_t c4_own, uint32_t c4_rest, uint32_t cap, void *scratch,
                                         const float4 *sums, const float4 *recv, hipStream_t s)
{
    const PlaneScratch v = plane_scratch(scratch, a.n_total);
    return launch_ring_finish_phase_kernel(a, np, ga, wpb, c4_own, c4_rest, cap, v.flags, v.px, v.py, v.pz, (float *)v.behind, sums, recv,
                                           next_plane_generation(), s);
}

hipError_t launch_instances(uint32_t count, const float4 *pos, const float4 *vel, float4 *inst, hipStream_t s, uint32_t device_libm)
{
    hipLaunchKernelGGL(instances_kernel, dim3(ceil_div(count, kBlock)), dim3(kBlock), 0, s, count, pos, vel, inst, device_libm);
    return hipGetLastError();
}

hipError_t launch_pack(uint32_t count, const float *xyz, float4 *rec, hipStream_t s)
{
    hipLaunchKernelGGL(pack_kernel, dim3(ceil_div(count, kBlock)), dim3(kBlock), 0, s, count, xyz, rec);
    return hipGetLastError();
}

hipError_t launch_unpack(uint32_t count, const float4 *rec, float *xyz, hipStream_t s)
{
    hipLaunchKernelGGL(unpack_kernel, dim3(ceil_div(count, kBlock)), dim3(kBlock), 0, s, count, rec, xyz);
    return hipGetLastError();
}
// ... 18 lines not shown
```

nenbody_amd/csrc/nb_nbody_bc.inc:

```

#if defined(NB_EXP_BC_WAVES)
constexpr int kBcWaves = NB_EXP_BC_WAVES;
#else
constexpr int kBcWaves = 12;
#endif
constexpr int kBcThreads = kBcWaves * 64;
constexpr int kBcBlock = 64;
constexpr int kBcBlock3d = 32;
constexpr uint32_t kBcSpinBudget = 1u << 24;
static_assert(kBcBlock == kPlanePad, "planes are padded to whole blocks");

__global__ __launch_bounds__(kBlock) void planes_kernel(uint32_t n, uint32_t npad, const float4 *__restrict__ pos, float *__restrict__ px,
                                                        float *__restrict__ py, float *__restrict__ pz, uint32_t *__restrict__ flags,
                                                        uint32_t lo_bits, uint32_t hi_bits, uint32_t force, uint32_t generation)
{
    const uint32_t j = blockIdx.x * (uint32_t)kBlock + threadIdx.x;
    uint32_t f = force;
    if (j < npad) {
        const float4 r = j < n ? pos[j] : make_float4(0.f, 0.f, 0.f, 0.f);
        px[j] = r.x;
        py[j] = r.y;
        pz[j] = r.z;
        const uint32_t span = hi_bits - lo_bits;
        f |= coord_oor(r.x, lo_bits, span) | coord_oor(r.y, lo_bits, span) | coord_oor(r.z, lo_bits, span) | nonzero_bits(r.z);
    }
    f = wave_or(f);
    if ((threadIdx.x & 63) == 0) {
        if (f & kFlagIeee) flags[kBcFlagWordIeee] = generation;
        if (f & kFlagNonPlanar) flags[kBcFlagWordNonPlanar] = generation;
    }
}

__global__ __launch_bounds__(kBlock) void planes_range_kernel(uint32_t n, const float4 *__restrict__ pos, float *__restrict__ px,
                                                              float *__restrict__ py, float *__restrict__ pz, uint32_t *__restrict__ flags,
                                                              uint32_t r0, uint32_t r1, uint32_t f0, uint32_t f1, uint32_t lo_bits,
                                                              uint32_t hi_bits, uint32_t force, uint32_t generation)
{
    const uint32_t j = blockIdx.x * (uint32_t)kBlock + threadIdx.x;
    uint32_t f = force;
    if (j < n && ((j >= r0 && j < r1) || (j >= f0 && j < f1))) {
        const float4 r = pos[j];
        px[j] = r.x;
        py[j] = r.y;
        pz[j] = r.z;
        const uint32_t span = hi_bits - lo_bits;
        f |= coord_oor(r.x, lo_bits, span) | coord_oor(r.y, lo_bits, span) | coord_oor(r.z, lo_bits, span) | nonzero_bits(r.z);
    }
    f = wave_or(f);
    if ((threadIdx.x & 63) == 0) {
        if (f & kFlagIeee) flags[kBcFlagWordIeee] = generation;
        if (f & kFlagNonPlanar) flags[kBcFlagWordNonPlanar] = generation;
    }
}

__global__ __launch_bounds__(kBlock) void ring_planes_kernel(uint32_t n, const float4 *__restrict__ pos, float *__restrict__ px,
                                                             float *__restrict__ py, float *__restrict__ pz, uint32_t *__restrict__ flags,
                                                             uint32_t r0, uint32_t r1, uint32_t generation, const uint32_t *move_from,
                                                             uint32_t *move_to)
{
    if (move_from && blockIdx.x == 0 && threadIdx.x < 3u) move_to[threadIdx.x] = move_from[threadIdx.x];
    const uint32_t j = r0 + blockIdx.x * (uint32_t)kBlock + threadIdx.x;
    uint32_t f = 0u;
    if (j < r1 && j < n) {
        const float4 r = pos[j];
        px[j] = r.x;
        py[j] = r.y;
        pz[j] = r.z;
        constexpr uint32_t span = 0x4d7fffffu;
        f |= coord_oor(r.x, 0u, span) | coord_oor(r.y, 0u, span) | coord_oor(r.z, 0u, span) | nonzero_bits(r.z);
    }
    f = wave_or(f);
    if ((threadIdx.x & 63) == 0) {
        if (f & kFlagIeee) flags[kBcFlagWordIeee] = generation;
        if (f & kFlagNonPlanar) flags[kBcFlagWordNonPlanar] = generation;
        if (blockIdx.x == 0 && threadIdx.x == 0) flags[kRingGenWord] = generation;
// ... 201 lines not shown
    BcSharedLds &sh = *(BcSharedLds *)(uintptr_t)uniform_u32(sh_lds);
    uint32_t gave_up = 0u;
    bc_run<true, false, kBcBlock3d>(c, uniform_ptr(px), uniform_ptr(py), uniform_ptr(pz), sh, (int)uniform_u32((uint32_t)wave), lane, xi, yi,
                                    zi, uniform_u32(budget_per_wait), gave_up);
    return gave_up;
}

__global__ __launch_bounds__(kBcThreads) void step_strict_bc_kernel(StepArgs a, const uint32_t *__restrict__ flags, uint32_t generation,
                                                                    const float *__restrict__ px, const float *__restrict__ py,
                                                                    const float *__restrict__ pz, uint32_t *__restrict__ status)
{
    __shared__ BcShared sh;
    const int tid = threadIdx.x;
    const int wave = __builtin_amdgcn_readfirstlane(tid >> 6);
    const int lane = tid & 63;
    const uint32_t l = blockIdx.x * 64u + (uint32_t)lane;
    const bool live = l < a.count;
    const float4 pi = a.pos_in[a.first + (live ? l : a.count - 1u)];
    if (tid < 64) {
        sh.sum[0][tid] = 0.f;
        sh.sum[1][tid] = 0.f;
        sh.sum[2][tid] = 0.f;
#if defined(NB_BC_HANDOFF64)
        sh.st[0][tid] = sh.st[1][tid] = sh.st[2][tid] = 0ull;
#endif
    }
    if (tid == 0) {
        sh.turn[0] = sh.turn[1] = sh.turn[2] = 0u;
        sh.gave_up = 0u;
    }
    __syncthreads();
    const uint32_t f = ((uint32_t)__builtin_amdgcn_readfirstlane(flags[kBcFlagWordIeee]) == generation ? kFlagIeee : 0u) |
                       ((uint32_t)__builtin_amdgcn_readfirstlane(flags[kBcFlagWordNonPlanar]) == generation ? kFlagNonPlanar : 0u) | a.force_ieee |
                       a.force_3d;
    const uint32_t budget_per_wait = a.spin_budget ? a.spin_budget : kBcSpinBudget;
    uint32_t gave_up = 0u;
    const BcConsts c{a.n_total, a.G, a.bias, a.bc_prio};
    if (f & kFlagIeee)
        gave_up = bc_run_ieee(a.n_total, a.G, a.bias, px, py, pz, (uint32_t)(uintptr_t)(BcSharedLds *)&sh, wave, lane, pi.x, pi.y, pi.z,
                              budget_per_wait, a.bc_prio);
    else if (f == 0u)
#if defined(NB_EXP_BC_PLANAR_BLOCK)
        bc_run<false, true, NB_EXP_BC_PLANAR_BLOCK>(c, px, py, pz, sh, wave, lane, pi.x, pi.y, pi.z, budget_per_wait, gave_up);
#else
        bc_run<false, true, kBcBlock>(c, px, py, pz, sh, wave, lane, pi.x, pi.y, pi.z, budget_per_wait, gave_up);
#endif
    else
        bc_run<false, false, kBcBlock3d>(c, px, py, pz, sh, wave, lane, pi.x, pi.y, pi.z, budget_per_wait, gave_up);
    if (gave_up && lane == 0) {
        sh.gave_up = 1u;
        atomicOr(status, 1u);
    }
    __syncthreads();
    if (wave == 0 && live) {
        float4 p = pi;
        float4 v = a.vel[l];
#if defined(NB_BC_HANDOFF64)
        integrate(p, v, __uint_as_float((uint32_t)sh.st[0][lane]), __uint_as_float((uint32_t)sh.st[1][lane]), __uint_as_float((uint32_t)sh.st[2][lane]), a.dt);
#else
        integrate(p, v, sh.sum[0][lane], sh.sum[1][lane], sh.sum[2][lane], a.dt);
#endif
        if (sh.gave_up) p.x = p.y = p.z = v.x = v.y = v.z = __builtin_nanf("");
        a.vel[l] = v;
        a.pos_out[a.first + l] = p;
    }
}
```

nenbody_amd/csrc/nb_nbody_sl.inc:

```

typedef float v8f __attribute__((ext_vector_type(8)));
typedef float v16f __attribute__((ext_vector_type(16)));

template <int G>
struct SlRecs {
    float x[G], y[G], z[G];
};
template <int G>
struct SlQuot {
    v2f x[G / 2], y[G / 2], z[G / 2];
};

template <bool PLANAR, int G>
__device__ __forceinline__ void sl_request(SlRecs<G> &r, const float *__restrict__ px, const float *__restrict__ py,
                                           const float *__restrict__ pz, uint32_t off)
{
    static_assert(G == 8 || G == 16, "one s_load_dwordx8 / x16 per plane");
    using V = typename std::conditional<G == 16, v16f, v8f>::type;
    const V vx = *reinterpret_cast<const V *>(reinterpret_cast<const char *>(px) + off);
    const V vy = *reinterpret_cast<const V *>(reinterpret_cast<const char *>(py) + off);
#pragma unroll
    for (int i = 0; i < G; ++i) r.x[i] = vx[i], r.y[i] = vy[i];
    if (!PLANAR) {
        const V vz = *reinterpret_cast<const V *>(reinterpret_cast<const char *>(pz) + off);
// ... 107 lines not shown
        sl_request<PLANAR, G>(rb, px, py, pz, off);
        __builtin_amdgcn_sched_barrier(0);
        q = sl_group<IEEE, PLANAR, G>(c, ra, q, xi, yi, zi, Gc, bias, sx, sy, sz);
        __builtin_amdgcn_sched_barrier(0);
        __builtin_amdgcn_s_waitcnt(0xC07F);
        off += kBytes;
        sl_request<PLANAR, G>(ra, px, py, pz, off);
        __builtin_amdgcn_sched_barrier(0);
        q = sl_group<IEEE, PLANAR, G>(c, rb, q, xi, yi, zi, Gc, bias, sx, sy, sz);
        __builtin_amdgcn_sched_barrier(0);
    }
    if (g < full) {
        q = sl_group<IEEE, PLANAR, G>(c, ra, q, xi, yi, zi, Gc, bias, sx, sy, sz);
        ++g;
        off += kBytes;
        sl_request<PLANAR, G>(ra, px, py, pz, off);
    }
#pragma unroll
    for (int k = 0; k < G; ++k) sl_add<PLANAR, G>(q, k / 2, k & 1, sx, sy, sz);
    const uint32_t left = n - g * (uint32_t)G;
    if (left) {
#pragma unroll
        for (int j = 0; j < G - 1; ++j) {
            if ((uint32_t)j < left) {
                float qx, qy, qz;
                pair_strict<IEEE, PLANAR>(make_float4(ra.x[j], ra.y[j], PLANAR ? 0.f : ra.z[j], bias), xi, yi, zi, Gc, qx, qy, qz);
                sx = sx + qx;
                sy = sy + qy;
                if (!PLANAR) sz = sz + qz;
            }
        }
    }
}

template <int W, int GP>
__global__ __launch_bounds__(64 * W) __attribute__((amdgpu_waves_per_eu(1, 2))) void step_strict_sl_kernel(
    StepArgs a, const uint32_t *__restrict__ flags, uint32_t generation, const float *__restrict__ px, const float *__restrict__ py,
    const float *__restrict__ pz)
{
    const ClockStamp stamp0 = clock_begin(a.stamps);
    const uint32_t l = blockIdx.x * (uint32_t)(64 * W) + threadIdx.x;
    const bool live = l < a.count;
    const float4 pi = a.pos_in[a.first + (live ? l : a.count - 1u)];
    const uint32_t f = ((uint32_t)__builtin_amdgcn_readfirstlane(flags[kBcFlagWordIeee]) == generation ? kFlagIeee : 0u) |
                       ((uint32_t)__builtin_amdgcn_readfirstlane(flags[kBcFlagWordNonPlanar]) == generation ? kFlagNonPlanar : 0u) | a.force_ieee |
                       a.force_3d;
    float sx = 0.f, sy = 0.f, sz = 0.f;
    if (f & kFlagIeee)
        sl_run<true, false, 8>(a.n_total, a.G, a.bias, px, py, pz, pi.x, pi.y, pi.z, sx, sy, sz);
    else if (f == 0u)
        sl_run<false, true, GP>(a.n_total, a.G, a.bias, px, py, pz, pi.x, pi.y, pi.z, sx, sy, sz);
    else
        sl_run<false, false, 8>(a.n_total, a.G, a.bias, px, py, pz, pi.x, pi.y, pi.z, sx, sy, sz);
    if (live) {
        float4 p = pi;
        float4 v = a.vel[l];
        integrate(p, v, sx, sy, sz, a.dt);
        a.vel[l] = v;
        a.pos_out[a.first + l] = p;
    }
    clock_end(a.stamps, stamp0);
}

hipError_t launch_strict_sl_kernel(const StepArgs &a, uint32_t shape, const uint32_t *flags, uint32_t generation, const float *px,
                                   const float *py, const float *pz, hipStream_t s)
{
#ifdef NB_LEGACY_FORMS
    if (shape == 2) {
        hipLaunchKernelGGL((step_strict_sl_kernel<1, 8>), dim3((a.count + 63u) / 64u), dim3(64), 0, s, a, flags, generation, px, py, pz);
        return hipGetLastError();
    }
    if (shape == 1) {
        hipLaunchKernelGGL((step_strict_sl_kernel<4, 8>), dim3((a.count + 255u) / 256u), dim3(256), 0, s, a, flags, generation, px, py, pz);
        return hipGetLastError();
    }
#else
    if (shape == 1 || shape == 2) return hipErrorNotSupported;
#endif
    hipLaunchKernelGGL((step_strict_sl_kernel<4, 16>), dim3((a.count + 255u) / 256u), dim3(256), 0, s, a, flags, generation, px, py, pz);
    return hipGetLastError();
}

template <int IB>
struct FslState {
    v2f xi[IB], yi[IB], zi[IB];
    v2f ax[IB], ay[IB], az[IB];
};

template <bool PLANAR, bool SHARED, int IB>
__device__ __forceinline__ void fsl_pair(FslState<IB> &s, v2f xj, v2f yj, v2f zj, v2f bias2)
{
    v2f dx[IB], dy[IB], dz[IB], r2[IB], inv[IB];
#define NBK_ROW _Pragma("unroll") for (int b = 0; b < IB; ++b)
    NBK_ROW dx[b] = xj - s.xi[b];
    NBK_ROW dy[b] = yj - s.yi[b];
    NBK_ROW r2[b] = __builtin_elementwise_fma(dx[b], dx[b], bias2);
    if (!PLANAR) {
        NBK_ROW dz[b] = zj - s.zi[b];
    }
    NBK_ROW r2[b] = __builtin_elementwise_fma(dy[b], dy[b], r2[b]);
    if (!PLANAR) {
        NBK_ROW r2[b] = __builtin_elementwise_fma(dz[b], dz[b], r2[b]);
    }
    if (SHARED) {
        float p[IB], rp[IB];
        NBK_ROW p[b] = r2[b].x * r2[b].y;
        NBK_ROW rp[b] = __builtin_amdgcn_rcpf(p[b]);
        NBK_ROW inv[b] = v2f{rp[b], rp[b]} * v2f{r2[b].y, r2[b].x};
    } else {
        NBK_ROW inv[b] = (v2f{__builtin_amdgcn_rcpf(r2[b].x), __builtin_amdgcn_rcpf(r2[b].y)});
    }
    NBK_ROW s.ax[b] = __builtin_elementwise_fma(dx[b], inv[b], s.ax[b]);
    NBK_ROW s.ay[b] = __builtin_elementwise_fma(dy[b], inv[b], s.ay[b]);
// ... 96 lines not shown
    const uint32_t r_lo = v_lo + a.j_base, r_hi = v_hi + a.j_base;
    uint32_t lo0 = r_lo, hi0 = r_hi, lo1 = 0u, hi1 = 0u;
    if (r_lo >= a.hole_lo) {
        lo0 = r_lo + a.hole_len, hi0 = r_hi + a.hole_len;
    } else if (r_hi > a.hole_lo) {
        hi0 = a.hole_lo;
        lo1 = a.hole_lo + a.hole_len, hi1 = r_hi + a.hole_len;
    }
    if (planar && share) {
        fsl_range<true, true, IB>(s, px, py, pz, lo0, hi0, a.bias);
        if (hi1 > lo1) fsl_range<true, true, IB>(s, px, py, pz, lo1, hi1, a.bias);
    } else if (planar) {
        fsl_range<true, false, IB>(s, px, py, pz, lo0, hi0, a.bias);
        if (hi1 > lo1) fsl_range<true, false, IB>(s, px, py, pz, lo1, hi1, a.bias);
    } else if (share) {
        fsl_range<false, true, IB>(s, px, py, pz, lo0, hi0, a.bias);
        if (hi1 > lo1) fsl_range<false, true, IB>(s, px, py, pz, lo1, hi1, a.bias);
    } else {
        fsl_range<false, false, IB>(s, px, py, pz, lo0, hi0, a.bias);
        if (hi1 > lo1) fsl_range<false, false, IB>(s, px, py, pz, lo1, hi1, a.bias);
    }

    float ax[IB], ay[IB], az[IB];
#pragma unroll
    for (int b = 0; b < IB; ++b) {
        ax[b] = s.ax[b].x + s.ax[b].y;
        ay[b] = s.ay[b].x + s.ay[b].y;
        az[b] = s.az[b].x + s.az[b].y;
    }
    if (W > 1) {
        if (w > 0) {
#pragma unroll
            for (int b = 0; b < IB; ++b) {
                part[w - 1][0][b * 64 + lane] = ax[b];
                part[w - 1][1][b * 64 + lane] = ay[b];
                part[w - 1][2][b * 64 + lane] = az[b];
            }
        }
        __syncthreads();
        if (w > 0) return;
#pragma unroll
        for (int g = 1; g < W; ++g) {
#pragma unroll
            for (int b = 0; b < IB; ++b) {
                ax[b] = ax[b] + part[g - 1][0][b * 64 + lane];
                ay[b] = ay[b] + part[g - 1][1][b * 64 + lane];
                az[b] = az[b] + part[g - 1][2][b * 64 + lane];
            }
        }
    }
#pragma unroll
    for (int b = 0; b < IB; ++b) {
        const uint32_t l = base + (uint32_t)(b * 64);
        if (l >= a.count) continue;
        if (gridDim.y == 1 && !a.always_partial) {
            float4 p = make_float4(s.xi[b].x, s.yi[b].x, s.zi[b].x, 0.f);
            float4 v = a.vel[l];
            integrate(p, v, ax[b] * a.G, ay[b] * a.G, az[b] * a.G, a.dt);
            a.vel[l] = v;
            a.pos_out[a.first + l] = p;
        } else {
            a.partial[(size_t)(a.partial_row0 + blockIdx.y) * a.count + l] = make_float4(ax[b], ay[b], az[b], 0.f);
        }
    }
    clock_end(a.stamps, stamp0);
}

hipError_t launch_fast_sl_kernel(const StepArgs &a, uint32_t ib, uint32_t slices, const uint32_t *flags, uint32_t generation,
                                 const float *px, const float *py, const float *pz, hipStream_t s)
{
#define NBK_FSL(I)                                                                                                             \
    if (ib == I) {                                                                                                             \
        hipLaunchKernelGGL((step_fast_sl_kernel<I, 8>), dim3((a.count + 64u * I - 1u) / (64u * I), slices), dim3(64 * 8), 0, s, a, flags, \
                           generation, px, py, pz);                                                                            \
        return hipGetLastError();                                                                                              \
    }
    NBK_FSL(4)
    NBK_FSL(2)
    NBK_FSL(1)
#undef NBK_FSL
    return hipErrorInvalidValue;
}
```

nenbody_amd/csrc/nb_nbody_strict.inc:

```

template <int TJ>
struct TileRegs {
    float4 r[TJ / kBlock];
};

template <int TJ>
__device__ __forceinline__ void tile_fetch(TileRegs<TJ> &t, const float4 *__restrict__ pos, uint32_t j0, uint32_t jend,
                                           int tid)
{
#pragma unroll
    for (int k = 0; k < TJ / kBlock; ++k) {
        const uint32_t j = j0 + (uint32_t)(k * kBlock + tid);
        t.r[k] = (j < jend) ? pos[j] : make_float4(0.f, 0.f, 0.f, 0.f);
    }
}

template <int TJ>
__device__ __forceinline__ void tile_store(const TileRegs<TJ> &t, float4 *lds_tile, int tid, float bias)
{
#pragma unroll
    for (int k = 0; k < TJ / kBlock; ++k)
        lds_tile[k * kBlock + tid] = make_float4(t.r[k].x, t.r[k].y, t.r[k].z, bias);
}

// ... 137 lines not shown
    for (; g + S <= nj; g += S) {
        float qx, qy, qz;
        pair_strict<IEEE, PLANAR>(tile[g + sl], xi, yi, zi, G, qx, qy, qz);
        add_in_lane_order<S>(sx, qx);
        add_in_lane_order<S>(sy, qy);
        if (!PLANAR) add_in_lane_order<S>(sz, qz);
    }
    if (S > 1 && g < nj) {
        const bool valid = g + sl < nj;
        float qx, qy, qz;
        pair_strict<IEEE, PLANAR>(tile[valid ? g + sl : g], xi, yi, zi, G, qx, qy, qz);
        qx = valid ? qx : 0.f;
        qy = valid ? qy : 0.f;
        qz = valid ? qz : 0.f;
        add_in_lane_order<S>(sx, qx);
        add_in_lane_order<S>(sy, qy);
        if (!PLANAR) add_in_lane_order<S>(sz, qz);
    }
}

__device__ __forceinline__ void integrate(float4 &p, float4 &v, float ax, float ay, float az, float dt)
{
    const float ex = ax * dt, ey = ay * dt, ez = az * dt;
    v.x = v.x + ex;
    v.y = v.y + ey;
    v.z = v.z + ez;
    p.x = v.x + p.x;
    p.y = v.y + p.y;
    p.z = v.z + p.z;
    p.w = 0.f;
    v.w = 0.f;
}

constexpr uint32_t kFlagIeee = 1u;
constexpr uint32_t kFlagNonPlanar = 2u;

__device__ __forceinline__ uint32_t wave_or(uint32_t v)
{
    return (__any((int)(v & kFlagIeee)) ? kFlagIeee : 0u) | (__any((int)(v & kFlagNonPlanar)) ? kFlagNonPlanar : 0u);
}

__device__ __forceinline__ uint32_t nonzero_bits(float c) { return (__float_as_uint(c) & 0x7fffffffu) != 0u ? kFlagNonPlanar : 0u; }

constexpr int kPlanePad = 64;
constexpr uint32_t kBcFlagsBytes = 256;
constexpr int kBcFlagWordIeee = 0;
constexpr int kBcFlagWordNonPlanar = 1;
constexpr int kRingGenWord = 2;
constexpr int kRingFlagsOwn = 8;
constexpr int kRingFlagsRest = 16;
constexpr int kRingFlagsNext = 24;
static_assert((kRingFlagsNext + kRingGenWord + 1) * sizeof(uint32_t) <= kBcFlagsBytes, "the phases' flag words fit the flags area");
__host__ __device__ inline uint32_t bc_padded(uint32_t n) { return (n + (uint32_t)kPlanePad - 1u) / (uint32_t)kPlanePad * (uint32_t)kPlanePad; }

typedef float v2f __attribute__((ext_vector_type(2)));
constexpr int kPackedUnroll = 4;

struct Pack2Consts {
    v2f xi, yi, zi, g, bias, one;
};

__device__ __forceinline__ Pack2Consts pack2_consts(float xi, float yi, float zi, float G, float bias)
{
    return Pack2Consts{{xi, xi}, {yi, yi}, {zi, zi}, {G, G}, {bias, bias}, {1.0f, 1.0f}};
}

template <bool PLANAR>
__device__ __forceinline__ void pair2_strict(const Pack2Consts &c, v2f xj, v2f yj, v2f zj, v2f &qx, v2f &qy, v2f &qz)
{
    const v2f dx = xj - c.xi, dy = yj - c.yi;
    const v2f xx = dx * dx, yy = dy * dy;
    v2f d, dz = {0.f, 0.f};
    if (PLANAR) {
        d = (xx + yy) + c.bias;
    } else {
        dz = zj - c.zi;
        const v2f zz = dz * dz;
        d = ((xx + yy) + zz) + c.bias;
    }
    const v2f nx = dx * c.g, ny = dy * c.g;
    const v2f r0 = {__builtin_amdgcn_rcpf(d.x), __builtin_amdgcn_rcpf(d.y)};
    const v2f e = __builtin_elementwise_fma(-d, r0, c.one);
    const v2f r = __builtin_elementwise_fma(e, r0, r0);
    const v2f q0x = nx * r, q0y = ny * r;
    const v2f t0x = __builtin_elementwise_fma(-d, q0x, nx), t0y = __builtin_elementwise_fma(-d, q0y, ny);
    qx = __builtin_elementwise_fma(t0x, r, q0x);
    qy = __builtin_elementwise_fma(t0y, r, q0y);
    if (PLANAR) {
        qz = v2f{0.f, 0.f};
    } else {
        const v2f nz = dz * c.g, q0z = nz * r;
        const v2f t0z = __builtin_elementwise_fma(-d, q0z, nz);
        qz = __builtin_elementwise_fma(t0z, r, q0z);
    }
}

template <bool PLANAR, int U>
__device__ __forceinline__ void fold_tile_packed(const float *px, const float *py, const float *pz, int nj, float xi, float yi,
                                                 float zi, float G, float bias, float &sx, float &sy, float &sz)
{
    static_assert(U % 4 == 0, "groups of four j's per ds_read_b128");
    constexpr int Q = U / 4;
    const Pack2Consts c = pack2_consts(xi, yi, zi, G, bias);
    auto eval2 = [&](v2f xj, v2f yj, v2f zj) {
        v2f qx, qy, qz;
        pair2_strict<PLANAR>(c, xj, yj, zj, qx, qy, qz);
// ... 171 lines not shown
```

nenbody_amd/csrc/nb_nbody_sym.inc:

```
constexpr int pr_block(int np) { return 128 * np; }

template <int kNP>
struct PrState {
    v2f xi[kNP], yi[kNP], zi[kNP];
    v2f ax[kNP], ay[kNP], az[kNP];
};

__device__ __forceinline__ float pr_rotate_sub(float acc, float t)
{
    return __int_as_float(__builtin_amdgcn_update_dpp(0, __float_as_int(acc), 0x134 , 0xf, 0xf, false)) - t;
}
__device__ __forceinline__ float pr_rotate(float acc)
{
    return __int_as_float(__builtin_amdgcn_update_dpp(0, __float_as_int(acc), 0x134, 0xf, 0xf, false));
}

template <bool PLANAR, bool SHARED, int K, int kNP>
__device__ __forceinline__ void pr_steps(PrState<kNP> &s, const float (&bx)[K], const float (&by)[K], const float (&bz)[K], v2f bias2, float &sx,
                                         float &sy, float &sz)
{
    v2f dx[K][kNP], dy[K][kNP], dz[K][kNP], r2[K][kNP], inv[K][kNP], tx[K], ty[K], tz[K];
#define NBK_ROW _Pragma("unroll") for (int k = 0; k < K; ++k) _Pragma("unroll") for (int b = 0; b < kNP; ++b)
#define NBK_ROWK _Pragma("unroll") for (int k = 0; k < K; ++k)
    NBK_ROW dx[k][b] = v2f{bx[k], bx[k]} - s.xi[b];
// ... 255 lines not shown
    const bool planar = (f & kFlagNonPlanar) == 0u;
    const uint32_t lo = P * (uint32_t)kPrSuper + (uint32_t)w * (uint32_t)kPrBlock;
    const uint32_t j_lo = lo < n ? lo : n, j_hi = lo + (uint32_t)kPrBlock < n ? lo + (uint32_t)kPrBlock : n;
    if (planar && share)
        fsl_range<true, true, IB>(s, px, py, pz, j_lo, j_hi, a.bias);
    else if (planar)
        fsl_range<true, false, IB>(s, px, py, pz, j_lo, j_hi, a.bias);
    else if (share)
        fsl_range<false, true, IB>(s, px, py, pz, j_lo, j_hi, a.bias);
    else
        fsl_range<false, false, IB>(s, px, py, pz, j_lo, j_hi, a.bias);
    float ax[IB], ay[IB], az[IB];
#pragma unroll
    for (int b = 0; b < IB; ++b) {
        ax[b] = s.ax[b].x + s.ax[b].y;
        ay[b] = s.ay[b].x + s.ay[b].y;
        az[b] = s.az[b].x + s.az[b].y;
    }
    if (kPrW > 1) {
        if (w > 0) {
#pragma unroll
            for (int b = 0; b < IB; ++b) {
                part[w - 1][0][b * 64 + lane] = ax[b];
                part[w - 1][1][b * 64 + lane] = ay[b];
                part[w - 1][2][b * 64 + lane] = az[b];
            }
        }
        __syncthreads();
        if (w > 0) return;
#pragma unroll
        for (int g = 1; g < kPrW; ++g) {
#pragma unroll
            for (int b = 0; b < IB; ++b) {
                ax[b] = ax[b] + part[g - 1][0][b * 64 + lane];
                ay[b] = ay[b] + part[g - 1][1][b * 64 + lane];
                az[b] = az[b] + part[g - 1][2][b * 64 + lane];
            }
        }
    }
    const size_t plane = (size_t)tl.ra * tl.la;
    float *const row = tl.rows_a + (size_t)(P - tl.p0) * tl.la + (base - tl.a0);
#pragma unroll
    for (int b = 0; b < IB; ++b) {
        row[64 * b] = ax[b];
        row[plane + 64 * b] = ay[b];
        if (!planar) row[2 * plane + 64 * b] = az[b];
    }
}

__global__ __launch_bounds__(256) void pairs_integrate_kernel(StepArgs a, const uint32_t *__restrict__ flags, uint32_t generation,
                                                              const float *__restrict__ rows, uint32_t ns)
{
    const uint32_t l = blockIdx.x * 256u + threadIdx.x;
    if (l >= a.count) return;
    const bool planar = (flags[kBcFlagWordNonPlanar] != generation) && !a.force_3d;
    const size_t plane = (size_t)ns * a.n_total;
    float sx = 0.f, sy = 0.f, sz = 0.f;
    const float *r = rows + l;
    for (uint32_t k = 0; k < ns; ++k, r += a.n_total) {
        sx = sx + r[0];
        sy = sy + r[plane];
        if (!planar) sz = sz + r[2 * plane];
    }
    float4 p = a.pos_in[l];
    float4 v = a.vel[l];
    integrate(p, v, sx * a.G, sy * a.G, sz * a.G, a.dt);
    a.vel[l] = v;
    a.pos_out[l] = p;
}

__global__ __launch_bounds__(256) void pairs_accumulate_kernel(const uint32_t *__restrict__ flags, uint32_t generation, uint32_t force_3d,
                                                               float *__restrict__ acc, uint32_t n, const float *__restrict__ rows, uint32_t r_,
                                                               uint32_t len, uint32_t first, uint32_t fresh)
{
    const uint32_t l = blockIdx.x * 256u + threadIdx.x;
    if (l >= len || first + l >= n) return;
    const bool planar = (flags[kBcFlagWordNonPlanar] != generation) && !force_3d;
    const size_t plane = (size_t)r_ * len;
    float *const dst = acc + first + l;
    float sx = fresh ? 0.f : dst[0], sy = fresh ? 0.f : dst[n], sz = (fresh || planar) ? 0.f : dst[2 * (size_t)n];
    const float *r = rows + l;
    for (uint32_t k = 0; k < r_; ++k, r += len) {
        sx = sx + r[0];
        sy = sy + r[plane];
        if (!planar) sz = sz + r[2 * plane];
    }
    dst[0] = sx;
    dst[n] = sy;
    if (!planar) dst[2 * (size_t)n] = sz;
}
__global__ __launch_bounds__(256) void pairs_finish_kernel(StepArgs a, const uint32_t *__restrict__ flags, uint32_t generation,
                                                           const float *__restrict__ acc)
{
    const uint32_t l = blockIdx.x * 256u + threadIdx.x;
    if (l >= a.count) return;
    const bool planar = (flags[kBcFlagWordNonPlanar] != generation) && !a.force_3d;
    const float sx = acc[l], sy = acc[a.n_total + l], sz = planar ? 0.f : acc[2 * (size_t)a.n_total + l];
    float4 p = a.pos_in[l];
    float4 v = a.vel[l];
    integrate(p, v, sx * a.G, sy * a.G, sz * a.G, a.dt);
    a.vel[l] = v;
    a.pos_out[l] = p;
}

constexpr uint32_t kPrOneTileMax = 262144u;
constexpr uint32_t kPrChunk = 131072u;
uint32_t fast_pairs_chunk(uint32_t n_total, uint32_t chunk) { return chunk ? chunk : n_total <= kPrOneTileMax ? n_total : kPrChunk; }
size_t fast_pairs_scratch_floats(uint32_t n_total, uint32_t w, uint32_t np, uint32_t chunk)
{
    const uint32_t c = fast_pairs_chunk(n_total, chunk), super = (uint32_t)pr_block((int)np) * w;
    const size_t rows = (size_t)3 * ((c + super - 1u) / super) * c;
    return c >= n_total ? rows : (size_t)3 * n_total + 2 * rows;
}

template <int W, int NP>
static hipError_t launch_fast_pairs_w(const StepArgs &a, uint32_t chunk, const uint32_t *flags, uint32_t generation, const float *px,
                                      const float *py, const float *pz, float *scratch, hipStream_t s)
{
    constexpr uint32_t kPrBlock = (uint32_t)pr_block(NP);
    const uint32_t super = kPrBlock * W, n = a.n_total;
    auto tile = [&](uint32_t a0, uint32_t la, uint32_t b0, uint32_t lb, float *rows_a, float *rows_b) -> hipError_t {
        PrTile tl{};
        tl.p0 = a0 / super, tl.np = (la + super - 1u) / super, tl.a0 = a0, tl.la = la;
        tl.q0 = b0 / super, tl.nq = (lb + super - 1u) / super, tl.b0 = b0, tl.lb = lb;
        tl.rect = a0 != b0;
        tl.rows_a = rows_a, tl.rows_b = rows_b;
        tl.ra = tl.rect ? tl.nq : tl.np, tl.rb = tl.np;
        if (!tl.rect) {
            hipLaunchKernelGGL((pairs_diag_kernel<W, NP>), dim3(la / kPrBlock), dim3(64 * W), 0, s, a, flags, generation, px, py, pz, tl);
            if (tl.np > 1u)
                hipLaunchKernelGGL((step_fast_pairs_kernel<W, NP>), dim3(tl.np * (tl.np - 1u) / 2u), dim3(64 * W), 0, s, a, flags, generation, px, py, pz, tl);
        } else {
            hipLaunchKernelGGL((step_fast_pairs_kernel<W, NP>), dim3(tl.np * tl.nq), dim3(64 * W), 0, s, a, flags, generation, px, py, pz, tl);
        }
        return hipGetLastError();
    };
    if (chunk >= n) {
        hipError_t e = tile(0, n, 0, n, scratch, scratch);
        if (e != hipSuccess) return e;
        hipLaunchKernelGGL(pairs_integrate_kernel, dim3((a.count + 255u) / 256u), dim3(256), 0, s, a, flags, generation, scratch, (n + super - 1u) / super);
        return hipGetLastError();
    }
    float *const acc = scratch;
    const size_t rows_floats = (size_t)3 * ((chunk + super - 1u) / super) * chunk;
    float *const rows_a = acc + (size_t)3 * n, *const rows_b = rows_a + rows_floats;
    auto accumulate = [&](const float *rows, uint32_t r_, uint32_t len, uint32_t first, bool fresh) {
        hipLaunchKernelGGL(pairs_accumulate_kernel, dim3((len + 255u) / 256u), dim3(256), 0, s, flags, generation, a.force_3d, acc, n, rows, r_, len, first,
                           fresh ? 1u : 0u);
    };
    for (uint32_t a0 = 0; a0 < n; a0 += chunk) {
        const uint32_t la = n - a0 < chunk ? n - a0 : chunk, npa = (la + super - 1u) / super;
        hipError_t e = tile(a0, la, a0, la, rows_a, rows_a);
        if (e != hipSuccess) return e;
        accumulate(rows_a, npa, la, a0, a0 == 0);
        for (uint32_t b0 = a0 + chunk; b0 < n; b0 += chunk) {
// ... 34 lines not shown
```

nenbody_amd/csrc/nb_selftest.inc:

```


NB_EXPORT int nb_selftest_divide(const nb_params *params, uint64_t pairs, uint64_t seed, uint64_t *mismatches, float *bad_pair)
{
    if (!mismatches) {
        g_tls_error = "nb_selftest_divide: mismatches is null";
        return NB_ERR_INVALID;
    }
    nb_params p = params_or_default(params);
    p.mode = NB_MODE_STRICT;
    Plan pl;
    int rc = make_plan(p, 1024, 1024, &pl, &g_tls_error);
    if (rc != NB_OK) return rc;
    if (pl.guard.force_ieee && !overrides().strict_force_ieee.on()) {
        g_tls_error = "nb_selftest_divide: these parameters have no guarded range (STRICT always divides with '/')";
        return NB_ERR_UNSUPPORTED;
    }
    if (pl.guard.force_ieee) {
        g_tls_error = "nb_selftest_divide: unset NB_STRICT_FORCE_IEEE";
        return NB_ERR_UNSUPPORTED;
    }
    rc = check_device(&g_tls_error);
    if (rc != NB_OK) return rc;
    const int d_lo = pl.guard.c, d_hi = std::max(2 * pl.guard.b + 4, pl.guard.c + 2) - 1;
    const int n_lo = pl.guard.a - 23 + pl.guard.g, n_hi = pl.guard.b + pl.guard.g + 1;
// ... 280 lines not shown
    if (e1) (void)hipEventDestroy(e1);
    if (e != hipSuccess || !(ms > 0.f)) {
        g_tls_error = std::string("nb_selftest_valu_rate: ") + hipGetErrorString(e);
        return NB_ERR_HIP;
    }
    *lane_ops_per_s = (mix == 2 ? 128.0 : 64.0) * (double)trips * 256.0 * (double)blocks / ((double)ms * 1e-3);
    return NB_OK;
}

NB_EXPORT int nb_diag_step_clock(const nb_params *params, uint32_t n, double seconds, double *clock_mhz, double *wave_cycles,
                                 double *kernel_ms)
{
    if (!clock_mhz || !(seconds > 0.0) || seconds > 5.0 || n == 0) {
        g_tls_error = "nb_diag_step_clock: need clock_mhz != NULL, n > 0 and 0 < seconds <= 5";
        return NB_ERR_INVALID;
    }
    nb_params p = params_or_default(params);
    Plan pl;
    int rc = make_plan(p, n, n, &pl, &g_tls_error);
    if (rc != NB_OK) return rc;
    if (!pl.stamped) {
        g_tls_error = "nb_diag_step_clock: only the whole-set kernels carry stamps (STRICT one lane per body, FAST wave and pairs forms)";
        return NB_ERR_UNSUPPORTED;
    }
    nb_ctx *c = nullptr;
    rc = nb_create(n, 1, &p, &c);
    if (rc != NB_OK) return rc;
    std::vector<float> pos((size_t)n * 3), vel((size_t)n * 3);
    nb_init_state(1234, n, pos.data(), vel.data());
    rc = nb_upload(c, pos.data(), vel.data());
    const size_t groups = nbp::stamp_groups(pl, n, KernelSizes{});
    unsigned long long *stamps = nullptr;
    hipEvent_t e0 = nullptr, e1 = nullptr;
    hipError_t e = hipSuccess;
    float ms = 0.f;
    if (rc == NB_OK) {
        e = hipMalloc((void **)&stamps, groups * 4 * sizeof(unsigned long long));
        if (e == hipSuccess) e = hipMemsetAsync(stamps, 0, groups * 4 * sizeof(unsigned long long), c->stream);
        if (e == hipSuccess) e = hipEventCreate(&e0);
        if (e == hipSuccess) e = hipEventCreate(&e1);
        if (e == hipSuccess) rc = nb_step(c, 1);
        if (e == hipSuccess && rc == NB_OK) e = hipEventRecord(e0, c->stream);
        if (e == hipSuccess && rc == NB_OK) rc = nb_step(c, 1);
        if (e == hipSuccess && rc == NB_OK) e = hipEventRecord(e1, c->stream);
        if (e == hipSuccess && rc == NB_OK) e = hipEventSynchronize(e1);
        if (e == hipSuccess && rc == NB_OK) e = hipEventElapsedTime(&ms, e0, e1);
        if (e == hipSuccess && rc == NB_OK && ms > 0.f) {
            const uint32_t k = (uint32_t)std::min(std::max(seconds * 1e3 / (double)ms, 2.0), 100000.0);
            rc = nb_step(c, k - 1u);
            if (rc == NB_OK) e = hipEventRecord(e0, c->stream);
            if (rc == NB_OK && e == hipSuccess) {
                nbk::StepArgs a = step_args(p, pl, n, 0, n, c->pos[c->cur].p, c->pos[c->cur ^ 1].p, c->vel.p, c->scratch.p);
                a.stamps = stamps;
                e = launch_planned(pl, a, c->scratch.p, nullptr, c->stream);
            }
            if (rc == NB_OK && e == hipSuccess) e = hipEventRecord(e1, c->stream);
            if (rc == NB_OK && e == hipSuccess) e = hipEventSynchronize(e1);
            if (rc == NB_OK && e == hipSuccess) e = hipEventElapsedTime(&ms, e0, e1);
        }
    }
    double mhz = 0.0, cycles = 0.0;
    if (rc == NB_OK && e == hipSuccess) {
        std::vector<unsigned long long> st(groups * 4);
        e = hipMemcpy(st.data(), stamps, st.size() * sizeof(unsigned long long), hipMemcpyDeviceToHost);
        if (e == hipSuccess && !clock_from_stamps(st, &mhz, &cycles)) {
            g_tls_error = "nb_diag_step_clock: no workgroup ran long enough to time";
            rc = NB_ERR_STATE;
        }
    }
    if (rc != NB_OK && c) g_tls_error = c->err.empty() ? g_tls_error : c->err;
    if (stamps) (void)hipFree(stamps);
    if (e0) (void)hipEventDestroy(e0);
    if (e1) (void)hipEventDestroy(e1);
    nb_destroy(c);
    if (rc != NB_OK) return rc;
    if (e != hipSuccess) {
        g_tls_error = std::string("nb_diag_step_clock: ") + hipGetErrorString(e);
        return NB_ERR_HIP;
    }
    *clock_mhz = mhz;
    if (wave_cycles) *wave_cycles = cycles;
    if (kernel_ms) *kernel_ms = (double)ms;
    return NB_OK;
}
```

nenbody_amd/dist.py:

```python
from __future__ import annotations

import contextlib
import ctypes
import time
from typing import List, Optional, Tuple

import numpy as np

from . import _lib
from ._lib import NbParams, check

__all__ = ["partition", "ShardedScene", "HipBackend", "NativeShard", "comm_id"]


def partition(n: int, world: int) -> List[Tuple[int, int]]:
    if n <= 0 or world <= 0:
        raise ValueError("partition needs n > 0 and world > 0")
    slot = -(-n // world)
    out = []
    for r in range(world):
        first = min(r * slot, n)
        out.append((first, max(0, min(n - first, slot))))
    return out


class HipBackend:

    name = "hip"

    def __init__(self):
        self.lib = _lib.load()

    def scratch_bytes(self, params: NbParams, n_total: int, count: int) -> int:
        return int(self.lib.nb_scratch_bytes(ctypes.byref(params), n_total, count))

    @staticmethod
    def _launch(anchor, call, scope=True) -> None:
        import torch

        stream = torch.cuda.current_stream(anchor.device).cuda_stream
        with torch.cuda.device(anchor.device) if scope else contextlib.nullcontext():
            check(call(stream))

    def step(self, params, n_total, first, count, pos_in, pos_out, vel, scratch) -> None:
        sp = scratch.data_ptr() if scratch is not None and scratch.numel() else None
        sb = scratch.numel() if scratch is not None else 0
        self._launch(pos_in, lambda stream: self.lib.nb_launch_step(
            ctypes.byref(params), n_total, first, count, pos_in.data_ptr(), pos_out.data_ptr(), vel.data_ptr(), sp, sb, stream))

    def scratch_bytes_phased(self, params: NbParams, n_total: int, count: int, j_lo: int, j_hi: int) -> int:
        return int(self.lib.nb_scratch_bytes_phased(ctypes.byref(params), n_total, count, j_lo, j_hi))

    def step_phase(self, params, n_total, first, count, j_lo, j_hi, phase, pos_in, pos_out, vel, scratch) -> None:
        self._launch(pos_in, lambda stream: self.lib.nb_launch_step_phase(
            ctypes.byref(params), n_total, first, count, j_lo, j_hi, phase, pos_in.data_ptr(), pos_out.data_ptr(), vel.data_ptr(),
            scratch.data_ptr(), scratch.numel(), stream))

    def ring_partners(self, params: NbParams, n_total: int, first: int, count: int) -> int:
        d = int(self.lib.nb_ring_partners(ctypes.byref(params), n_total, first, count))
        if d < 0:
            check(d)
        return d

    def ring_scratch_bytes(self, params: NbParams, n_total: int, first: int, count: int) -> int:
        return int(self.lib.nb_ring_scratch_bytes(ctypes.byref(params), n_total, first, count))

    def ring_fold(self, params, n_total, first, count, pos_in, sums, scratch) -> None:
        self._launch(pos_in, lambda stream: self.lib.nb_launch_ring_fold(
            ctypes.byref(params), n_total, first, count, pos_in.data_ptr(), sums.data_ptr(), scratch.data_ptr(), scratch.numel(), stream))

    def ring_phased(self, params: NbParams, n_total: int, first: int, count: int) -> bool:
        r = int(self.lib.nb_ring_phased(ctypes.byref(params), n_total, first, count))
        if r < 0:
            check(r)
        return r == 1

    def ring_fold_phase(self, params, n_total, first, count, phase, pos_in, sums, scratch) -> None:
        self._launch(pos_in, lambda stream: self.lib.nb_launch_ring_fold_phase(
            ctypes.byref(params), n_total, first, count, int(phase), pos_in.data_ptr(), sums.data_ptr(), scratch.data_ptr(),
            scratch.numel(), stream))

    def ring_finish(self, params, n_total, first, count, pos_in, pos_out, vel, sums, recv) -> None:
        self._launch(pos_in, lambda stream: self.lib.nb_launch_ring_finish(
            ctypes.byref(params), n_total, first, count, pos_in.data_ptr(), pos_out.data_ptr(), vel.data_ptr(), sums.data_ptr(),
            recv.data_ptr(), stream))

    def ring_finish_phase(self, params, n_total, first, count, pos_in, pos_out, vel, sums, recv, scratch) -> None:
        self._launch(pos_in, lambda stream: self.lib.nb_launch_ring_finish_phase(
            ctypes.byref(params), n_total, first, count, pos_in.data_ptr(), pos_out.data_ptr(), vel.data_ptr(),
            sums.data_ptr() if sums is not None else None, recv.data_ptr(), scratch.data_ptr(), scratch.numel(), stream))

    def instances(self, count, pos, vel, inst) -> None:
        self._launch(pos, lambda stream: self.lib.nb_launch_instances(count, pos.data_ptr(), vel.data_ptr(), inst.data_ptr(), stream),
                     scope=False)

    def boids_step(self, params, n_total, first, count, pos_in, vel_in, pos_out, vel_out) -> None:
        self._launch(pos_in, lambda stream: self.lib.nb_launch_boids_step(
            ctypes.byref(params), n_total, first, count, pos_in.data_ptr(), vel_in.data_ptr(), pos_out.data_ptr(), vel_out.data_ptr(),
            stream), scope=False)

    def boids_split_scratch_bytes(self, params, n_total, count) -> int:
# ... 10 lines not shown
    def __init__(self, positions, velocities, params: Optional[NbParams] = None, *, device=None, group=None,
                 backend=None, rank: Optional[int] = None, world: Optional[int] = None, overlap: bool = False,
                 ring: Optional[bool] = None, ring_overlap: Optional[bool] = None, exchange: str = "collective"):
        import torch
        import torch.distributed as dist

        self.torch = torch
        self.dist = dist
        self.group = group
        if world is None:
            world = dist.get_world_size(group) if dist.is_available() and dist.is_initialized() else 1
        if rank is None:
            rank = dist.get_rank(group) if world > 1 else 0
        self.world, self.rank = world, rank
        pos = np.ascontiguousarray(positions, dtype=np.float32)
        vel = np.ascontiguousarray(velocities, dtype=np.float32)
        if pos.ndim != 2 or pos.shape[1] != 3 or pos.shape != vel.shape:
            raise ValueError("positions and velocities must both have shape (n, 3)")
        self.n = len(pos)
        self.params = params if params is not None else _lib.default_params()
        self.backend = backend if backend is not None else HipBackend()
        if device is None:
            if self.backend.name == "hip":
                if not torch.cuda.is_available():
                    raise _lib.NbError(_lib.NB_ERR_NO_DEVICE, "no HIP device visible to torch; nenbody_amd has no CPU path")
                device = torch.device("cuda", torch.cuda.current_device())
            else:
                device = torch.device("cpu")
        self.device = torch.device(device)
        parts = partition(self.n, world)
        self.first, self.count = parts[rank]
        self.slot = -(-self.n // world)
        padded = self.slot * world
        rec = torch.zeros((padded, 4), dtype=torch.float32)
        rec[: self.n, :3] = torch.from_numpy(pos)
        self.pos = [rec.to(self.device), torch.zeros((padded, 4), dtype=torch.float32, device=self.device)]
        vrec = torch.zeros((max(self.count, 1), 4), dtype=torch.float32)
        if self.count:
            vrec[: self.count, :3] = torch.from_numpy(vel[self.first:self.first + self.count])
        self.vel = vrec.to(self.device)
        self.partners = 0
        if ring is not False and world > 1 and self.params.mode == _lib.NB_MODE_FAST and self.n == self.slot * world \
                and hasattr(self.backend, "ring_partners"):
            self.partners = self.backend.ring_partners(self.params, self.n, self.first, self.count)
        if ring and not self.partners:
            raise ValueError("ring=True: this shape does not take the pairs form on shards (FAST, equal ranks of whole blocks)")
        self.sums = self.recv = None
        if self.partners:
            self.sums = torch.zeros(((self.partners + 1) * self.count, 4), dtype=torch.float32, device=self.device)
            self.recv = torch.zeros((self.partners * self.count, 4), dtype=torch.float32, device=self.device)
        self.overlap = bool(overlap) and self.params.mode == _lib.NB_MODE_FAST and world > 1 and not self.partners
        self._pending = None
        self._own_ready = None
        can = bool(self.partners) and hasattr(self.backend, "ring_phased") and self.backend.ring_phased(self.params, self.n, self.first, self.count)
        if ring_overlap and not can:
            raise ValueError("ring_overlap=True: this shape does not run its step in phases (nb_ring_phased() == 0)")
        self.ring_overlap = can and bool(overlap if ring_overlap is None else ring_overlap)
        if self.partners:
            sb = self.backend.ring_scratch_bytes(self.params, self.n, self.first, self.count)
        elif self.overlap:
            sb = self.backend.scratch_bytes_phased(self.params, self.n, self.count, self.first, self.first + self.count) if self.count else 0
        else:
            sb = self.backend.scratch_bytes(self.params, self.n, self.count) if self.count else 0
        self.scratch = torch.empty((sb,), dtype=torch.uint8, device=self.device) if sb else None
        self.cur = 0
        self.steps_done = 0
        self.gather_in_place = True
        self.ring_grouped = True
        self.exchange_report = None
        self._collective_verdict = None
        self.exchange = "collective"
        self._peers = None
        self._peers_sums = False
        if exchange not in ("collective", "peers"):
            raise ValueError('exchange must be "collective" or "peers"')
        if exchange == "peers" and world > 1:
            if not self.setup_peers():
                raise _lib.NbError(_lib.NB_ERR_STATE, "exchange=\"peers\": the ranks could not map each other's buffers (" + str(self.peers_error) + ")")
            self.exchange = "peers"
        self.velfull = None
        self._pvstage = None
        self.velfull_valid = False

    def setup_peers(self) -> bool:
        torch, dist = self.torch, self.dist
        self.peers_error = None
        if self._peers is not None:
            return True
        lib = self.backend.lib if hasattr(self.backend, "lib") else None
        handle, ok = ctypes.c_void_p(), lib is not None and self.device.type == "cuda" and self.world <= 16
        every = None
        if not ok:
            self.peers_error = "needs the HIP backend, device buffers and at most 16 ranks"
        blob = ctypes.create_string_buffer(int(lib.nb_peers_blob_bytes())) if lib is not None else None
        if ok:
            with torch.cuda.device(self.device):
                bufs = [self.pos[0], self.pos[1]] + ([self.sums] if self.sums is not None else [])
                rc = lib.nb_peers_create(self.rank, self.world, ctypes.byref(handle))
                if rc == _lib.NB_OK:
                    ptrs = (ctypes.c_void_p * len(bufs))(*[b.data_ptr() for b in bufs])
                    sizes = (ctypes.c_size_t * len(bufs))(*[b.numel() * b.element_size() for b in bufs])
                    rc = lib.nb_peers_export(handle, ptrs, sizes, len(bufs), blob)
                if rc != _lib.NB_OK:
                    ok, self.peers_error = False, lib.nb_peers_last_error(handle if handle else None).decode()
        every = [None] * self.world
        dist.all_gather_object(every, blob.raw if ok else b"", group=self.group)
        if ok and all(len(e) == len(blob.raw) for e in every):
            joined = b"".join(every)
            with torch.cuda.device(self.device):
                rc = lib.nb_peers_import(handle, ctypes.create_string_buffer(joined, len(joined)))
            if rc != _lib.NB_OK:
                ok, self.peers_error = False, lib.nb_peers_last_error(handle).decode()
        elif ok:
            ok, self.peers_error = False, "another rank could not export its buffers"
# ... 211 lines not shown
        psrc, pdst = self.pos[self.cur], self.pos[self.cur ^ 1]
        vsrc, vdst = self.velfull[self.cur], self.velfull[self.cur ^ 1]
        if self.world > 1:
            if self._pvstage is None:
                self._pvstage = torch.zeros((self.world * 2 * self.slot, 4), dtype=torch.float32, device=self.device)
            st = self._pvstage
            if self.count:
                boids(bp, self.n, self.first, self.count, psrc, vsrc, st[self.rank * self.slot:], st[self.rank * self.slot + self.slot:])
            self._all_gather_slots(st, slot=2 * self.slot)
            both = st.view(self.world, 2, self.slot, 4)
            pdst.view(self.world, self.slot, 4).copy_(both[:, 0])
            vdst.view(self.world, self.slot, 4).copy_(both[:, 1])
        elif self.count:
            boids(bp, self.n, self.first, self.count, psrc, vsrc, pdst, vdst)
        if self.count:
            self.vel[: self.count] = vdst[lo:lo + self.count]
        self.cur ^= 1
        self.steps_done += 1

    def step(self) -> None:
        src, dst = self.pos[self.cur], self.pos[self.cur ^ 1]
        ready, self._own_ready = self._own_ready is not None and self._own_ready is self.scratch, None
        if self.partners and self.ring_overlap:
            be, a = self.backend, (self.params, self.n, self.first, self.count)
            be.ring_fold_phase(*a, _lib.NB_RING_OWN_READY if ready else _lib.NB_RING_OWN, src, self.sums, self.scratch)
            self._wait_pending()
            be.ring_fold_phase(*a, _lib.NB_RING_REST, src, self.sums, self.scratch)
            started = self._ring_exchange_start()
            in_stream = self.exchange == "peers" and self._peers_sums
            if not in_stream:
                be.ring_fold_phase(*a, _lib.NB_RING_SUMS, src, self.sums, self.scratch)
            self._ring_exchange_wait(started)
            be.ring_finish_phase(*a, src, dst, self.vel, None if in_stream else self.sums, self.recv, self.scratch)
            self._own_ready = self.scratch
            self._pending = self._all_gather_slots(dst, async_op=True)
        elif self.partners:
            self._wait_pending()
            self.backend.ring_fold(self.params, self.n, self.first, self.count, src, self.sums, self.scratch)
            self._ring_exchange()
            self.backend.ring_finish(self.params, self.n, self.first, self.count, src, dst, self.vel, self.sums, self.recv)
            self._all_gather_slots(dst)
        elif self.overlap:
            lo, hi = self.first, self.first + self.count
            if self.count:
                self.backend.step_phase(self.params, self.n, self.first, self.count, lo, hi, _lib.NB_PHASE_RANGE, src, dst, self.vel,
                                        self.scratch)
            self._wait_pending()
            if self.count:
                self.backend.step_phase(self.params, self.n, self.first, self.count, lo, hi, _lib.NB_PHASE_REST, src, dst, self.vel,
                                        self.scratch)
            self._pending = self._all_gather_slots(dst, async_op=True)
        else:
            self._wait_pending()
            if self.count:
                self.backend.step(self.params, self.n, self.first, self.count, src, dst, self.vel, self.scratch)
            if self.world > 1:
                self._all_gather_slots(dst)
        self.velfull_valid = False
        self.cur ^= 1
        self.steps_done += 1

    def step_n(self, k: int) -> None:
        for _ in range(int(k)):
            self.step()

    def choose_form(self, steps: int = 4, warm: int = 2) -> str:
        torch = self.torch
        self.form_times = None
        if not self.partners:
            return "ordered"
        self._wait_pending()
        saved = (self.pos[0].clone(), self.pos[1].clone(), self.vel.clone(), self.cur, self.steps_done, self.velfull_valid)
        sb = self.backend.scratch_bytes(self.params, self.n, self.count) if self.count else 0
        phased = hasattr(self.backend, "ring_phased") and self.backend.ring_phased(self.params, self.n, self.first, self.count)
        cands = {"pairs": (self.partners, self.scratch, False)}
        if phased:
            cands["pairs_overlapped"] = (self.partners, self.scratch, True)
        cands["ordered"] = (0, torch.empty((sb,), dtype=torch.uint8, device=self.device) if sb else None, False)

        def fence():
            self._wait_pending()
            if self.device.type == "cuda":
                torch.cuda.synchronize(self.device)
            self.dist.barrier(group=self.group)

        def restore():
            self._wait_pending()
            self.pos[0].copy_(saved[0])
            self.pos[1].copy_(saved[1])
            self.vel.copy_(saved[2])
            self.cur, self.steps_done, self.velfull_valid = saved[3], saved[4], saved[5]
            self._own_ready = None

        names, times = list(cands), []
        for name in names:
            self.partners, self.scratch, self.ring_overlap = cands[name]
            self.step_n(warm)
            fence()
            t0 = time.perf_counter()
            self.step_n(steps)
            fence()
            times.append((time.perf_counter() - t0) / max(1, steps))
            restore()
        on_device = self.dist.get_backend(self.group) == "nccl"
        t = torch.tensor(times, dtype=torch.float64, device=self.device if on_device else "cpu")
        self.dist.all_reduce(t, op=self.dist.ReduceOp.MAX, group=self.group)
        self.form_times = dict(zip(names, (float(x) for x in t.tolist())))
# ... 254 lines not shown
```

Before: 23.49 million.

## Chain plane layout from one step's integrate into the next step's force pass

The integrate kernels now also write the new positions into split x/y/z planes and range/planarity flags held in a second scratch area. When consecutive steps are chained and the input is unchanged, the next step reuses those planes instead of running a separate pass to build them. PlaneChain tracks validity per context and per scratch buffer, and any import, random step or error invalidates it. This costs extra scratch memory and extra stores in integrate, and stale chain state could give wrong results if an invalidation is missed.

```diff
diff --git a/include/nenbody.h b/include/nenbody.h
--- a/include/nenbody.h
+++ b/include/nenbody.h
@@ -162,6 +162,11 @@
 
 int nb_launch_step(const nb_params *params, uint32_t n_total, uint32_t first, uint32_t count, const void *pos_in,
                    void *pos_out, void *vel, void *scratch, size_t scratch_bytes, void *stream);
+
+enum { NB_STEP_CHAINED = 1 };
+size_t nb_chain_bytes(const nb_params *params, uint32_t n_total, uint32_t count);
+int nb_chain_step(const nb_params *params, uint32_t n_total, uint32_t first, uint32_t count, const void *pos_in,
+                           void *pos_out, void *vel, void *scratch, size_t scratch_bytes, uint32_t flags, void *stream);
 
 enum { NB_PHASE_RANGE = 0, NB_PHASE_REST = 1 };
 size_t nb_scratch_bytes_phased(const nb_params *params, uint32_t n_total, uint32_t count, uint32_t j_lo, uint32_t j_hi);
diff --git a/include/nenbody_diag.h b/include/nenbody_diag.h
--- a/include/nenbody_diag.h
+++ b/include/nenbody_diag.h
@@ -31,6 +31,8 @@
 
 int nb_diag_plan(const nb_params *params, uint32_t n_total, uint32_t count, char *out, size_t out_bytes);
 
+uint64_t nb_diag_planes_launches(void);
+
 #ifdef __cplusplus
 }
 #endif
diff --git a/nenbody_amd/_lib.py b/nenbody_amd/_lib.py
--- a/nenbody_amd/_lib.py
+++ b/nenbody_amd/_lib.py
@@ -20,6 +20,7 @@
 NB_MODE_FAST = 1
 NB_PHASE_RANGE = 0
 NB_PHASE_REST = 1
+NB_STEP_CHAINED = 1
 NB_RING_OWN, NB_RING_REST, NB_RING_SUMS, NB_RING_OWN_READY = 1, 2, 3, 4
 NB_SCENES_MAX_BODIES = 2048
 NB_EYES_NONE = 0xFFFFFFFF
@@ -154,6 +155,11 @@
         c_int,
         [POINTER(NbParams), c_uint32, c_uint32, c_uint32, c_void_p, c_void_p, c_void_p, c_void_p, c_size_t, c_void_p],
     ),
+    "nb_chain_bytes": (c_size_t, [POINTER(NbParams), c_uint32, c_uint32]),
+    "nb_chain_step": (
+        c_int,
+        [POINTER(NbParams), c_uint32, c_uint32, c_uint32, c_void_p, c_void_p, c_void_p, c_void_p, c_size_t, c_uint32, c_void_p],
+    ),
     "nb_scratch_bytes_phased": (c_size_t, [POINTER(NbParams), c_uint32, c_uint32, c_uint32, c_uint32]),
     "nb_launch_step_phase": (
         c_int,
@@ -241,6 +247,7 @@
     "nb_diag_legacy_forms": (c_int, []),
     "nb_diag_peers_lossy": (c_int, [c_int]),
     "nb_diag_plan": (c_int, [POINTER(NbParams), c_uint32, c_uint32, ctypes.c_char_p, c_size_t]),
+    "nb_diag_planes_launches": (c_uint64, []),
 }
 
 _lib = None
diff --git a/nenbody_amd/csrc/nb_api.hip b/nenbody_amd/csrc/nb_api.hip
--- a/nenbody_amd/csrc/nb_api.hip
+++ b/nenbody_amd/csrc/nb_api.hip
@@ -93,6 +93,12 @@
     size_t pairs_scratch_floats(uint32_t n, uint32_t w, uint32_t np, uint32_t chunk) const { return nbk::fast_pairs_scratch_floats(n, w, np, chunk); }
 };
 size_t plan_scratch_bytes(const Plan &pl, uint32_t count) { return nbp::plan_scratch_bytes(pl, count, KernelSizes{}); }
+size_t chained_second_at(const Plan &pl, uint32_t count) { return (plan_scratch_bytes(pl, count) + 255u) & ~(size_t)255u; }
+bool plan_chains(const Plan &pl, uint32_t count) { return nbp::form_info(pl.form).planes && count == pl.n_total; }
+size_t plan_scratch_bytes_chained(const Plan &pl, uint32_t count)
+{
+    return plan_chains(pl, count) ? chained_second_at(pl, count) + nbk::plane_set_bytes(pl.n_total) : plan_scratch_bytes(pl, count);
+}
 
 struct PlanKey {
     nb_params p;
@@ -290,18 +296,20 @@
     void *scratch;
     uint32_t *status;
     hipStream_t s;
+    const nbk::ChainArgs *chain;
     hipError_t strict(uint32_t tile, uint32_t unroll, uint32_t lanes) const { return nbk::launch_strict(a, tile, unroll, lanes, s); }
     hipError_t strict_pc(uint32_t producers) const { return nbk::launch_strict_pc(a, producers, s); }
-    hipError_t strict_bc() const { return nbk::launch_strict_bc(a, scratch, status, s); }
-    hipError_t strict_sl(uint32_t shape) const { return nbk::launch_strict_sl(a, shape, scratch, s); }
+    hipError_t strict_bc() const { return nbk::launch_strict_bc(a, scratch, status, s, chain); }
+    hipError_t strict_sl(uint32_t shape) const { return nbk::launch_strict_sl(a, shape, scratch, s, chain); }
     hipError_t fast(uint32_t tile, uint32_t ib, uint32_t groups, uint32_t slices) const { return nbk::launch_fast(a, tile, ib, groups, slices, s); }
     hipError_t fast_wave(uint32_t tile, uint32_t ib, uint32_t waves, uint32_t slices) const { return nbk::launch_fast_wave(a, tile, ib, waves, slices, s); }
-    hipError_t fast_sl(uint32_t ib, uint32_t slices) const { return nbk::launch_fast_sl(a, ib, slices, scratch, s); }
-    hipError_t fast_pairs(uint32_t w, uint32_t np, uint32_t chunk) const { return nbk::launch_fast_pairs(a, w, np, chunk, scratch, s); }
+    hipError_t fast_sl(uint32_t ib, uint32_t slices) const { return nbk::launch_fast_sl(a, ib, slices, scratch, s, chain); }
+    hipError_t fast_pairs(uint32_t w, uint32_t np, uint32_t chunk) const { return nbk::launch_fast_pairs(a, w, np, chunk, scratch, s, chain); }
 };
-hipError_t launch_planned(const Plan &pl, const nbk::StepArgs &a, void *scratch, uint32_t *status, hipStream_t stream)
-{
-    return nbp::visit_launch(pl, Launchers{a, scratch, status, stream});
+hipError_t launch_planned(const Plan &pl, const nbk::StepArgs &a, void *scratch, uint32_t *status, hipStream_t stream,
+                          const nbk::ChainArgs *chain = nullptr)
+{
+    return nbp::visit_launch(pl, Launchers{a, scratch, status, stream, chain});
 }
 
 int launch_status(hipError_t e, const char *what, std::string *err)
@@ -313,16 +321,18 @@
 
 int launch_step_planned(const nb_params &p, const Plan &pl, uint32_t n_total, uint32_t first, uint32_t count,
                         const void *pos_in, void *pos_out, void *vel, void *scratch, hipStream_t stream, std::string *err,
-                        StatusWord *sw = nullptr)
+                        StatusWord *sw = nullptr, nbp::PlaneChain *chain = nullptr, bool chain_asserted = false)
 {
     const nbk::StepArgs a = step_args(p, pl, n_total, first, count, pos_in, pos_out, vel, scratch);
+    const nbk::ChainArgs ca{chain, (chain && plan_chains(pl, count)) ? (char *)scratch + chained_second_at(pl, count) : nullptr, chain_asserted};
+    if (chain && !ca.second) chain->invalidate();
     uint32_t *status = nullptr;
     if (nbp::form_info(pl.form).status_word) {
         int rc = sw ? status_word_for_launch(sw, err) : device_status_word(&status, err);
         if (rc != NB_OK) return rc;
         if (sw) status = sw->w;
     }
-    hipError_t e = launch_planned(pl, a, scratch, status, stream);
+    hipError_t e = launch_planned(pl, a, scratch, status, stream, chain ? &ca : nullptr);
     if (e == hipErrorNotSupported) {
         *err = "nb: this launch shape is one of the legacy forms (NB_STRICT_PC / NB_STRICT_LANES / NB_STRICT_UNROLL / NB_STRICT_SL=2,3 / "
                "NB_FAST_WAVES / NB_FAST_GROUPS / NB_FAST_PAIRS_W): this library was built without them (make -C nenbody_amd/csrc legacy "
@@ -625,6 +635,7 @@
     uint32_t done_seq = 0, polled_calls = 0;
     uint32_t poll_holdoff = 0, poll_backoff = 0;
     DeviceBuffer<char> scratch;
+    nbp::PlaneChain chain;
     StatusWord status;
     int cur = 0;
     bool uploaded = false;
@@ -669,8 +680,9 @@
     return nbk::launch_instances(n, pos, vel, inst->p, stream, overrides().inst_device_libm.on() ? 1u : 0u);
 }
 
-static void step_done(nb_ctx *c, bool wrote_vel_alt)
-{
+static void step_done(nb_ctx *c, bool wrote_vel_alt, bool kept_planes = false)
+{
+    if (!kept_planes) c->chain.invalidate();
     c->cur ^= 1;
     if (wrote_vel_alt) c->vel.swap(c->vel_alt);
     c->steps++;
@@ -826,7 +838,7 @@
     NB_HIP(c, c->pos[1].reserve(c->n));
     NB_HIP(c, c->vel.reserve(c->n));
     NB_HIP(c, c->stage.reserve((size_t)c->n * 3));
-    NB_HIP(c, c->scratch.reserve(plan_scratch_bytes(c->plan, c->n)));
+    NB_HIP(c, c->scratch.reserve(plan_scratch_bytes_chained(c->plan, c->n)));
     return NB_OK;
 }
 
@@ -870,6 +882,7 @@
 static int small_import(nb_ctx *c, const float *pos_xyz, const float *vel_xyz)
 {
     const size_t n = c->n, bytes = n * 3 * sizeof(float);
+    c->chain.invalidate();
     std::memcpy(c->hxfer, pos_xyz, bytes);
     std::memcpy(c->hxfer + 3 * n, vel_xyz, bytes);
     float *src = c->hxfer_dev;
@@ -908,6 +921,7 @@
     }
     const size_t bytes = (size_t)ctx->n * 3 * sizeof(float);
     ctx->cur = 0;
+    ctx->chain.invalidate();
     if (ctx->n <= kRoundtripMax) {
         rc = ensure_xfer(ctx);
         if (rc != NB_OK) return rc;
@@ -937,9 +951,12 @@
     RoctxRange range("nb_step");
     for (uint32_t s = 0; s < k; ++s) {
         rc = launch_step_planned(ctx->p, ctx->plan, ctx->n, 0, ctx->n, ctx->pos[ctx->cur].p, ctx->pos[ctx->cur ^ 1].p, ctx->vel.p,
-                                 ctx->scratch.p, ctx->stream, &ctx->err, &ctx->status);
-        if (rc != NB_OK) return rc;
-        step_done(ctx, false);
+                                 ctx->scratch.p, ctx->stream, &ctx->err, &ctx->status, &ctx->chain, true);
+        if (rc != NB_OK) {
+            ctx->chain.invalidate();
+            return rc;
+        }
+        step_done(ctx, false, true);
     }
     return NB_OK;
 }
@@ -984,6 +1001,7 @@
     const int rc = ctx_check(ctx, "nb_step_random", kCallUpload);
     if (rc != NB_OK) return rc;
     for (uint32_t s = 0; s < k; ++s) {
+        ctx->chain.invalidate();
         NB_HIP(ctx, nbk::launch_random(0, ctx->n, ctx->pos[ctx->cur].p, ctx->vel.p, seed, ctx->steps, ctx->stream));
         ctx->steps++;
     }
@@ -1449,29 +1467,91 @@
     return plan_scratch_bytes(pl, count);
 }
 
+namespace {
+struct ScratchChains {
+    static constexpr int kAreas = 4;
+    const void *area[kAreas] = {};
+    nbp::PlaneChain chain[kAreas];
+    int next = 0;
+    nbp::PlaneChain *find(const void *scratch)
+    {
+        for (int i = 0; i < kAreas; ++i)
+            if (area[i] == scratch) return &chain[i];
+        return nullptr;
+    }
+    nbp::PlaneChain *get(const void *scratch)
+    {
+        if (nbp::PlaneChain *c = find(scratch)) return c;
+        const int i = next;
+        next = (next + 1) % kAreas;
+        area[i] = scratch;
+        chain[i] = nbp::PlaneChain{};
+        return &chain[i];
+    }
+};
+ScratchChains &scratch_chains()
+{
+    thread_local ScratchChains t;
+    return t;
+}
+
+int launch_step_api(const char *fn, const nb_params *params, uint32_t n_total, uint32_t first, uint32_t count, const void *pos_in, void *pos_out,
+                    void *vel, void *scratch, size_t scratch_bytes, bool chained_entry, uint32_t flags, void *stream)
+{
+    const nb_params p = params_or_default(params);
+    if (!pos_in || !pos_out || !vel || pos_in == pos_out) {
+        g_tls_error = std::string(fn) + ": pos_in, pos_out, vel must be non-null and pos_out must not alias pos_in";
+        return NB_ERR_INVALID;
+    }
+    if ((uint64_t)first + (uint64_t)count > (uint64_t)n_total) {
+        g_tls_error = std::string(fn) + ": [first, first+count) exceeds n_total";
+        return NB_ERR_INVALID;
+    }
+    if (flags & ~(uint32_t)NB_STEP_CHAINED) {
+        g_tls_error = std::string(fn) + ": unknown flag";
+        return NB_ERR_INVALID;
+    }
+    const Plan *pl = nullptr;
+    int rc = cached_plan(p, n_total, count, &pl, &g_tls_error);
+    if (rc != NB_OK) return rc;
+    const size_t need = chained_entry ? plan_scratch_bytes_chained(*pl, count) : plan_scratch_bytes(*pl, count);
+    if (need && (!scratch || scratch_bytes < need)) {
+        g_tls_error = std::string(fn) + (chained_entry ? ": scratch smaller than nb_chain_bytes()" : ": scratch smaller than nb_scratch_bytes()");
+        return NB_ERR_INVALID;
+    }
+    rc = device_for_launch(pos_in, stream, SelectDevice::kForNullStream);
+    if (rc != NB_OK) return rc;
+    nbp::PlaneChain *chain = nullptr;
+    if (scratch) {
+        chain = chained_entry ? scratch_chains().get(scratch) : scratch_chains().find(scratch);
+        if (chain && !chained_entry) chain->invalidate(), chain = nullptr;
+    }
+    rc = launch_step_planned(p, *pl, n_total, first, count, pos_in, pos_out, vel, scratch, (hipStream_t)stream, &g_tls_error, nullptr, chain,
+                             (flags & NB_STEP_CHAINED) != 0u);
+    if (rc != NB_OK && chain) chain->invalidate();
+    return rc;
+}
+}
+
 NB_EXPORT int nb_launch_step(const nb_params *params, uint32_t n_total, uint32_t first, uint32_t count, const void *pos_in,
                              void *pos_out, void *vel, void *scratch, size_t scratch_bytes, void *stream)
 {
+    return launch_step_api("nb_launch_step", params, n_total, first, count, pos_in, pos_out, vel, scratch, scratch_bytes, false, 0u, stream);
+}
+
+NB_EXPORT size_t nb_chain_bytes(const nb_params *params, uint32_t n_total, uint32_t count)
+{
     const nb_params p = params_or_default(params);
-    if (!pos_in || !pos_out || !vel || pos_in == pos_out) {
-        g_tls_error = "nb_launch_step: pos_in, pos_out, vel must be non-null and pos_out must not alias pos_in";
-        return NB_ERR_INVALID;
-    }
-    if ((uint64_t)first + (uint64_t)count > (uint64_t)n_total) {
-        g_tls_error = "nb_launch_step: [first, first+count) exceeds n_total";
-        return NB_ERR_INVALID;
-    }
-    const Plan *pl = nullptr;
-    int rc = cached_plan(p, n_total, count, &pl, &g_tls_error);
-    if (rc != NB_OK) return rc;
-    const size_t need = plan_scratch_bytes(*pl, count);
-    if (need && (!scratch || scratch_bytes < need)) {
-        g_tls_error = "nb_launch_step: scratch smaller than nb_scratch_bytes()";
-        return NB_ERR_INVALID;
-    }
-    rc = device_for_launch(pos_in, stream, SelectDevice::kForNullStream);
-    if (rc != NB_OK) return rc;
-    return launch_step_planned(p, *pl, n_total, first, count, pos_in, pos_out, vel, scratch, (hipStream_t)stream, &g_tls_error);
+    Plan pl;
+    std::string err;
+    if (make_plan(p, n_total, count, &pl, &err) != NB_OK) return 0;
+    return plan_scratch_bytes_chained(pl, count);
+}
+
+NB_EXPORT int nb_chain_step(const nb_params *params, uint32_t n_total, uint32_t first, uint32_t count, const void *pos_in,
+                                     void *pos_out, void *vel, void *scratch, size_t scratch_bytes, uint32_t flags, void *stream)
+{
+    return launch_step_api("nb_chain_step", params, n_total, first, count, pos_in, pos_out, vel, scratch, scratch_bytes, true, flags, stream);
 }
 
 NB_EXPORT int nb_launch_status(void *stream)
@@ -1601,6 +1681,8 @@
     return NB_OK;
 }
 
+NB_EXPORT uint64_t nb_diag_planes_launches(void) { return nbk::planes_launches(); }
+
 NB_EXPORT int nb_diag_plan(const nb_params *params, uint32_t n_total, uint32_t count, char *out, size_t out_bytes)
 {
     if (!out || out_bytes == 0) {
diff --git a/nenbody_amd/csrc/nb_chain.h b/nenbody_amd/csrc/nb_chain.h
--- /dev/null
+++ b/nenbody_amd/csrc/nb_chain.h
@@ -0,0 +1,41 @@
+#pragma once
+#include <stdint.h>
+
+namespace nbp {
+
+struct PlaneChain {
+    const void *pos = nullptr;
+    uint32_t n_total = 0, lo_bits = 0, hi_bits = 0;
+    uint32_t set = 0;
+    uint32_t gen = 0;
+
+    void invalidate() { pos = nullptr; }
+    bool holds(const void *pos_in, uint32_t n, uint32_t lo, uint32_t hi) const
+    {
+        return pos != nullptr && pos == pos_in && n_total == n && lo_bits == lo && hi_bits == hi;
+    }
+
+    struct Turn {
+        bool fill;
+        uint32_t set, gen, next_gen;
+    };
+    template <typename NextGen>
+    Turn begin(bool asserted, const void *pos_in, uint32_t n, uint32_t lo, uint32_t hi, NextGen next) const
+    {
+        Turn t;
+        t.fill = !(asserted && holds(pos_in, n, lo, hi));
+        t.set = t.fill ? 0u : set;
+        t.gen = t.fill ? next() : gen;
+        t.next_gen = next();
+        return t;
+    }
+    void done(const Turn &t, const void *pos_out, uint32_t n, uint32_t lo, uint32_t hi)
+    {
+        pos = pos_out;
+        n_total = n, lo_bits = lo, hi_bits = hi;
+        set = t.set ^ 1u;
+        gen = t.next_gen;
+    }
+};
+
+}
diff --git a/nenbody_amd/csrc/nb_kernels.h b/nenbody_amd/csrc/nb_kernels.h
--- a/nenbody_amd/csrc/nb_kernels.h
+++ b/nenbody_amd/csrc/nb_kernels.h
@@ -2,7 +2,16 @@
 #include <hip/hip_runtime.h>
 #include <stdint.h>
 
+#include "nb_chain.h"
+
 namespace nbk {
+
+struct NextPlanes {
+    float *px, *py, *pz;
+    uint32_t *flags;
+    uint32_t generation;
+    uint32_t lo_bits, hi_bits;
+};
 
 struct StepArgs {
     const float4 *pos_in;
@@ -22,6 +31,7 @@
     uint32_t partial_row0;
     uint32_t always_partial;
     unsigned long long *stamps;
+    NextPlanes next;
 };
 
 struct BoidsMaskK {
@@ -55,7 +65,14 @@
 hipError_t launch_strict(const StepArgs &a, uint32_t tile, uint32_t unroll, uint32_t lanes, hipStream_t s);
 hipError_t launch_strict_jp(const StepArgs &a, uint32_t tile, uint32_t unroll, uint32_t lanes, hipStream_t s);
 hipError_t launch_strict_pc(const StepArgs &a, uint32_t producers, hipStream_t s);
-hipError_t launch_strict_bc(const StepArgs &a, void *scratch, uint32_t *status, hipStream_t s);
+struct ChainArgs {
+    nbp::PlaneChain *chain;
+    void *second;
+    bool asserted;
+};
+size_t plane_set_bytes(uint32_t n_total);
+uint64_t planes_launches();
+hipError_t launch_strict_bc(const StepArgs &a, void *scratch, uint32_t *status, hipStream_t s, const ChainArgs *chain = nullptr);
 size_t strict_bc_scratch_bytes(uint32_t n_total);
 struct PlaneScratch {
     uint32_t *flags;
@@ -64,17 +81,18 @@
     uint32_t npad;
 };
 PlaneScratch plane_scratch(void *scratch, uint32_t n_total);
-hipError_t launch_strict_sl(const StepArgs &a, uint32_t shape, void *scratch, hipStream_t s);
+hipError_t launch_strict_sl(const StepArgs &a, uint32_t shape, void *scratch, hipStream_t s, const ChainArgs *chain = nullptr);
 hipError_t launch_strict_sl_kernel(const StepArgs &a, uint32_t shape, const uint32_t *flags, uint32_t generation, const float *px,
                                    const float *py, const float *pz, hipStream_t s);
 hipError_t launch_fast(const StepArgs &a, uint32_t tile, uint32_t ib, uint32_t groups, uint32_t slices, hipStream_t s);
 hipError_t launch_fast_wave(const StepArgs &a, uint32_t tile, uint32_t ib, uint32_t waves, uint32_t slices, hipStream_t s);
-hipError_t launch_fast_sl(const StepArgs &a, uint32_t ib, uint32_t slices, void *scratch, hipStream_t s);
+hipError_t launch_fast_sl(const StepArgs &a, uint32_t ib, uint32_t slices, void *scratch, hipStream_t s, const ChainArgs *chain = nullptr);
 hipError_t launch_fast_sl_phase(const StepArgs &a, uint32_t ib, uint32_t slices, bool range, uint32_t r0, uint32_t r1, void *scratch,
                                 hipStream_t s);
 hipError_t launch_fast_sl_kernel(const StepArgs &a, uint32_t ib, uint32_t slices, const uint32_t *flags, uint32_t generation,
                                  const float *px, const float *py, const float *pz, hipStream_t s);
-hipError_t launch_fast_pairs(const StepArgs &a, uint32_t w, uint32_t np, uint32_t chunk, void *scratch, hipStream_t s);
+hipError_t launch_fast_pairs(const StepArgs &a, uint32_t w, uint32_t np, uint32_t chunk, void *scratch, hipStream_t s,
+                             const ChainArgs *chain = nullptr);
 hipError_t launch_fast_pairs_kernels(const StepArgs &a, uint32_t w, uint32_t np, uint32_t chunk, const uint32_t *flags, uint32_t generation,
                                      const float *px, const float *py, const float *pz, float *scratch, hipStream_t s);
 uint32_t fast_pairs_rows(uint32_t n_total, uint32_t w, uint32_t np);
diff --git a/nenbody_amd/csrc/nb_launch.inc b/nenbody_amd/csrc/nb_launch.inc
--- a/nenbody_amd/csrc/nb_launch.inc
+++ b/nenbody_amd/csrc/nb_launch.inc
@@ -71,10 +71,65 @@
     return gen;
 }
 
-static void enqueue_planes(const StepArgs &a, const PlaneScratch &v, uint32_t lo_bits, uint32_t hi_bits, uint32_t gen, hipStream_t s)
-{
+static std::atomic<uint64_t> g_planes_launches{0};
+uint64_t planes_launches() { return g_planes_launches.load(std::memory_order_relaxed); }
+static void enqueue_planes(const StepArgs &a, const PlaneScratch &v, uint32_t lo_bits, uint32_t hi_bits, uint32_t gen, hipStream_t s,
+                           float *other = nullptr)
+{
+    g_planes_launches.fetch_add(1u, std::memory_order_relaxed);
     hipLaunchKernelGGL(planes_kernel, dim3(ceil_div(v.npad, kBlock)), dim3(kBlock), 0, s, a.n_total, v.npad, a.pos_in, v.px, v.py, v.pz,
-                       v.flags, lo_bits, hi_bits, 0u, gen);
+                       v.flags, lo_bits, hi_bits, 0u, gen, other);
+}
+
+size_t plane_set_bytes(uint32_t n_total) { return 3u * (size_t)bc_padded(n_total) * sizeof(float) + kPlaneSlackBytes; }
+struct PlanesOfLaunch {
+    const uint32_t *flags;
+    uint32_t gen;
+    const float *px, *py, *pz;
+    char *behind;
+    nbp::PlaneChain::Turn turn;
+    bool chained;
+};
+static hipError_t planes_of_launch(StepArgs &a, void *scratch, const ChainArgs *c, bool integrates, uint32_t lo_bits, uint32_t hi_bits,
+                                   hipStream_t s, PlanesOfLaunch *out)
+{
+    PlaneScratch v = plane_scratch(scratch, a.n_total);
+    out->behind = v.behind;
+    out->chained = c && c->chain && c->second && integrates && a.first == 0u && a.count == a.n_total;
+    if (!out->chained) {
+        if (c && c->chain) c->chain->invalidate();
+        out->gen = next_plane_generation();
+        enqueue_planes(a, v, lo_bits, hi_bits, out->gen, s);
+        out->flags = v.flags, out->px = v.px, out->py = v.py, out->pz = v.pz;
+        return hipGetLastError();
+    }
+    float *const x[2] = {v.px, (float *)c->second};
+    uint32_t *const fl[2] = {v.flags, v.flags + kChainFlagsAlt};
+    const nbp::PlaneChain::Turn t = c->chain->begin(c->asserted, a.pos_in, a.n_total, lo_bits, hi_bits, next_plane_generation);
+    out->turn = t;
+    if (t.fill) {
+        enqueue_planes(a, v, lo_bits, hi_bits, t.gen, s, x[1]);
+        const hipError_t e = hipGetLastError();
+        if (e != hipSuccess) {
+            c->chain->invalidate();
+            return e;
+        }
+    }
+    const uint32_t rd = t.set, wr = t.set ^ 1u;
+    out->flags = fl[rd], out->gen = t.gen;
+    out->px = x[rd], out->py = x[rd] + v.npad, out->pz = x[rd] + 2u * (size_t)v.npad;
+    a.next = NextPlanes{x[wr], x[wr] + v.npad, x[wr] + 2u * (size_t)v.npad, fl[wr], t.next_gen, lo_bits, hi_bits};
+    return hipSuccess;
+}
+static hipError_t planes_launched(const StepArgs &a, const ChainArgs *c, const PlanesOfLaunch &p, hipError_t e)
+{
+    if (p.chained) {
+        if (e == hipSuccess)
+            c->chain->done(p.turn, a.pos_out, a.n_total, a.next.lo_bits, a.next.hi_bits);
+        else
+            c->chain->invalidate();
+    }
+    return e;
 }
 constexpr uint32_t kFastPlaneLoBits = 0u, kFastPlaneHiBits = 0x4d7fffffu;
 static hipError_t launch_fast_planes(const StepArgs &a, const PlaneScratch &v, uint32_t gen, hipStream_t s)
@@ -83,24 +138,23 @@
     return hipGetLastError();
 }
 
-hipError_t launch_strict_bc(const StepArgs &a, void *scratch, uint32_t *status, hipStream_t s)
-{
-    const PlaneScratch v = plane_scratch(scratch, a.n_total);
-    const uint32_t gen = next_plane_generation();
-    enqueue_planes(a, v, a.lo_bits, a.hi_bits, gen, s);
-    hipLaunchKernelGGL(step_strict_bc_kernel, dim3(ceil_div(a.count, 64)), dim3(kBcThreads), 0, s, a, (const uint32_t *)v.flags, gen,
-                       (const float *)v.px, (const float *)v.py, (const float *)v.pz, status);
-    return hipGetLastError();
-}
-
-hipError_t launch_strict_sl(const StepArgs &a, uint32_t shape, void *scratch, hipStream_t s)
-{
-    const PlaneScratch v = plane_scratch(scratch, a.n_total);
-    const uint32_t gen = next_plane_generation();
-    enqueue_planes(a, v, a.lo_bits, a.hi_bits, gen, s);
-    hipError_t e = hipGetLastError();
-    if (e != hipSuccess) return e;
-    return launch_strict_sl_kernel(a, shape, v.flags, gen, v.px, v.py, v.pz, s);
+hipError_t launch_strict_bc(const StepArgs &a_in, void *scratch, uint32_t *status, hipStream_t s, const ChainArgs *chain)
+{
+    StepArgs a = a_in;
+    PlanesOfLaunch p;
+    hipError_t e = planes_of_launch(a, scratch, chain, true, a.lo_bits, a.hi_bits, s, &p);
+    if (e != hipSuccess) return e;
+    hipLaunchKernelGGL(step_strict_bc_kernel, dim3(ceil_div(a.count, 64)), dim3(kBcThreads), 0, s, a, p.flags, p.gen, p.px, p.py, p.pz, status);
+    return planes_launched(a, chain, p, hipGetLastError());
+}
+
+hipError_t launch_strict_sl(const StepArgs &a_in, uint32_t shape, void *scratch, hipStream_t s, const ChainArgs *chain)
+{
+    StepArgs a = a_in;
+    PlanesOfLaunch p;
+    hipError_t e = planes_of_launch(a, scratch, chain, true, a.lo_bits, a.hi_bits, s, &p);
+    if (e != hipSuccess) return e;
+    return planes_launched(a, chain, p, launch_strict_sl_kernel(a, shape, p.flags, p.gen, p.px, p.py, p.pz, s));
 }
 
 hipError_t launch_strict(const StepArgs &a, uint32_t tile, uint32_t unroll, uint32_t lanes, hipStream_t s)
@@ -206,15 +260,15 @@
     return hipErrorNotSupported;
 }
 
-hipError_t launch_fast_sl(const StepArgs &a_in, uint32_t ib, uint32_t slices, void *scratch, hipStream_t s)
-{
-    StepArgs a = a_in;
-    const PlaneScratch v = plane_scratch(scratch, a.n_total);
-    a.partial = (float4 *)v.behind;
-    const uint32_t gen = next_plane_generation();
-    hipError_t e = launch_fast_planes(a, v, gen, s);
-    if (e != hipSuccess) return e;
-    e = launch_fast_sl_kernel(a, ib, slices, v.flags, gen, v.px, v.py, v.pz, s);
+hipError_t launch_fast_sl(const StepArgs &a_in, uint32_t ib, uint32_t slices, void *scratch, hipStream_t s, const ChainArgs *chain)
+{
+    StepArgs a = a_in;
+    PlanesOfLaunch p;
+    const bool integrates = slices == 1 && !a.always_partial;
+    hipError_t e = planes_of_launch(a, scratch, chain, integrates, kFastPlaneLoBits, kFastPlaneHiBits, s, &p);
+    if (e != hipSuccess) return e;
+    a.partial = (float4 *)p.behind;
+    e = planes_launched(a, chain, p, launch_fast_sl_kernel(a, ib, slices, p.flags, p.gen, p.px, p.py, p.pz, s));
     if (e != hipSuccess || slices == 1 || a.always_partial) return e;
     return launch_integrate_partials(a, slices, s);
 }
@@ -238,13 +292,13 @@
     return launch_fast_sl_kernel(a, ib, slices, v.flags, gen, v.px, v.py, v.pz, s);
 }
 
-hipError_t launch_fast_pairs(const StepArgs &a, uint32_t w, uint32_t np, uint32_t chunk, void *scratch, hipStream_t s)
-{
-    const PlaneScratch v = plane_scratch(scratch, a.n_total);
-    const uint32_t gen = next_plane_generation();
-    hipError_t e = launch_fast_planes(a, v, gen, s);
-    if (e != hipSuccess) return e;
-    return launch_fast_pairs_kernels(a, w, np, chunk, v.flags, gen, v.px, v.py, v.pz, (float *)v.behind, s);
+hipError_t launch_fast_pairs(const StepArgs &a_in, uint32_t w, uint32_t np, uint32_t chunk, void *scratch, hipStream_t s, const ChainArgs *chain)
+{
+    StepArgs a = a_in;
+    PlanesOfLaunch p;
+    hipError_t e = planes_of_launch(a, scratch, chain, true, kFastPlaneLoBits, kFastPlaneHiBits, s, &p);
+    if (e != hipSuccess) return e;
+    return planes_launched(a, chain, p, launch_fast_pairs_kernels(a, w, np, chunk, p.flags, p.gen, p.px, p.py, p.pz, (float *)p.behind, s));
 }
 
 hipError_t launch_fast_ring(const StepArgs &a, uint32_t np, uint32_t ga, uint32_t wpb, void *scratch, float4 *sums, hipStream_t s)
diff --git a/nenbody_amd/csrc/nb_nbody_bc.inc b/nenbody_amd/csrc/nb_nbody_bc.inc
--- a/nenbody_amd/csrc/nb_nbody_bc.inc
+++ b/nenbody_amd/csrc/nb_nbody_bc.inc
@@ -12,7 +12,8 @@
 
 __global__ __launch_bounds__(kBlock) void planes_kernel(uint32_t n, uint32_t npad, const float4 *__restrict__ pos, float *__restrict__ px,
                                                         float *__restrict__ py, float *__restrict__ pz, uint32_t *__restrict__ flags,
-                                                        uint32_t lo_bits, uint32_t hi_bits, uint32_t force, uint32_t generation)
+                                                        uint32_t lo_bits, uint32_t hi_bits, uint32_t force, uint32_t generation,
+                                                        float *__restrict__ other)
 {
     const uint32_t j = blockIdx.x * (uint32_t)kBlock + threadIdx.x;
     uint32_t f = force;
@@ -21,6 +22,7 @@
         px[j] = r.x;
         py[j] = r.y;
         pz[j] = r.z;
+        if (other && j >= n) other[j] = other[npad + j] = other[2u * npad + j] = 0.f;
         const uint32_t span = hi_bits - lo_bits;
         f |= coord_oor(r.x, lo_bits, span) | coord_oor(r.y, lo_bits, span) | coord_oor(r.z, lo_bits, span) | nonzero_bits(r.z);
     }
@@ -328,16 +330,19 @@
         atomicOr(status, 1u);
     }
     __syncthreads();
-    if (wave == 0 && live) {
+    if (wave == 0) {
         float4 p = pi;
-        float4 v = a.vel[l];
+        if (live) {
+            float4 v = a.vel[l];
 #if defined(NB_BC_HANDOFF64)
-        integrate(p, v, __uint_as_float((uint32_t)sh.st[0][lane]), __uint_as_float((uint32_t)sh.st[1][lane]), __uint_as_float((uint32_t)sh.st[2][lane]), a.dt);
-#else
-        integrate(p, v, sh.sum[0][lane], sh.sum[1][lane], sh.sum[2][lane], a.dt);
-#endif
-        if (sh.gave_up) p.x = p.y = p.z = v.x = v.y = v.z = __builtin_nanf("");
-        a.vel[l] = v;
-        a.pos_out[a.first + l] = p;
-    }
-}
+            integrate(p, v, __uint_as_float((uint32_t)sh.st[0][lane]), __uint_as_float((uint32_t)sh.st[1][lane]), __uint_as_float((uint32_t)sh.st[2][lane]), a.dt);
+#else
+            integrate(p, v, sh.sum[0][lane], sh.sum[1][lane], sh.sum[2][lane], a.dt);
+#endif
+            if (sh.gave_up) p.x = p.y = p.z = v.x = v.y = v.z = __builtin_nanf("");
+            a.vel[l] = v;
+            a.pos_out[a.first + l] = p;
+        }
+        next_planes_store(a.next, live, a.first + l, p.x, p.y, p.z);
+    }
+}
diff --git a/nenbody_amd/csrc/nb_nbody_sl.inc b/nenbody_amd/csrc/nb_nbody_sl.inc
--- a/nenbody_amd/csrc/nb_nbody_sl.inc
+++ b/nenbody_amd/csrc/nb_nbody_sl.inc
@@ -183,13 +183,14 @@
         sl_run<false, true, GP>(a.n_total, a.G, a.bias, px, py, pz, pi.x, pi.y, pi.z, sx, sy, sz);
     else
         sl_run<false, false, 8>(a.n_total, a.G, a.bias, px, py, pz, pi.x, pi.y, pi.z, sx, sy, sz);
+    float4 p = pi;
     if (live) {
-        float4 p = pi;
         float4 v = a.vel[l];
         integrate(p, v, sx, sy, sz, a.dt);
         a.vel[l] = v;
         a.pos_out[a.first + l] = p;
     }
+    next_planes_store(a.next, live, a.first + l, p.x, p.y, p.z);
     clock_end(a.stamps, stamp0);
 }
 
@@ -392,14 +393,17 @@
 #pragma unroll
     for (int b = 0; b < IB; ++b) {
         const uint32_t l = base + (uint32_t)(b * 64);
-        if (l >= a.count) continue;
+        const bool live = l < a.count;
         if (gridDim.y == 1 && !a.always_partial) {
             float4 p = make_float4(s.xi[b].x, s.yi[b].x, s.zi[b].x, 0.f);
-            float4 v = a.vel[l];
-            integrate(p, v, ax[b] * a.G, ay[b] * a.G, az[b] * a.G, a.dt);
-            a.vel[l] = v;
-            a.pos_out[a.first + l] = p;
-        } else {
+            if (live) {
+                float4 v = a.vel[l];
+                integrate(p, v, ax[b] * a.G, ay[b] * a.G, az[b] * a.G, a.dt);
+                a.vel[l] = v;
+                a.pos_out[a.first + l] = p;
+            }
+            next_planes_store(a.next, live, a.first + l, p.x, p.y, p.z);
+        } else if (live) {
             a.partial[(size_t)(a.partial_row0 + blockIdx.y) * a.count + l] = make_float4(ax[b], ay[b], az[b], 0.f);
         }
     }
diff --git a/nenbody_amd/csrc/nb_nbody_strict.inc b/nenbody_amd/csrc/nb_nbody_strict.inc
--- a/nenbody_amd/csrc/nb_nbody_strict.inc
+++ b/nenbody_amd/csrc/nb_nbody_strict.inc
@@ -213,6 +213,26 @@
 constexpr int kRingFlagsNext = 24;
 static_assert((kRingFlagsNext + kRingGenWord + 1) * sizeof(uint32_t) <= kBcFlagsBytes, "the phases' flag words fit the flags area");
 __host__ __device__ inline uint32_t bc_padded(uint32_t n) { return (n + (uint32_t)kPlanePad - 1u) / (uint32_t)kPlanePad * (uint32_t)kPlanePad; }
+constexpr int kChainFlagsAlt = 4;
+static_assert(kChainFlagsAlt + kBcFlagWordNonPlanar < kRingFlagsOwn, "set 1's flag words are nobody else's");
+
+__device__ __forceinline__ void next_planes_store(const NextPlanes &nx, bool live, uint32_t j, float x, float y, float z)
+{
+    if (!nx.px) return;
+    uint32_t f = 0u;
+    if (live) {
+        nx.px[j] = x;
+        nx.py[j] = y;
+        nx.pz[j] = z;
+        const uint32_t span = nx.hi_bits - nx.lo_bits;
+        f = coord_oor(x, nx.lo_bits, span) | coord_oor(y, nx.lo_bits, span) | coord_oor(z, nx.lo_bits, span) | nonzero_bits(z);
+    }
+    f = wave_or(f);
+    if ((threadIdx.x & 63) == 0) {
+        if (f & kFlagIeee) nx.flags[kBcFlagWordIeee] = nx.generation;
+        if (f & kFlagNonPlanar) nx.flags[kBcFlagWordNonPlanar] = nx.generation;
+    }
+}
 
 typedef float v2f __attribute__((ext_vector_type(2)));
 constexpr int kPackedUnroll = 4;
diff --git a/nenbody_amd/csrc/nb_nbody_sym.inc b/nenbody_amd/csrc/nb_nbody_sym.inc
--- a/nenbody_amd/csrc/nb_nbody_sym.inc
+++ b/nenbody_amd/csrc/nb_nbody_sym.inc
@@ -331,21 +331,25 @@
                                                               const float *__restrict__ rows, uint32_t ns)
 {
     const uint32_t l = blockIdx.x * 256u + threadIdx.x;
-    if (l >= a.count) return;
-    const bool planar = (flags[kBcFlagWordNonPlanar] != generation) && !a.force_3d;
-    const size_t plane = (size_t)ns * a.n_total;
-    float sx = 0.f, sy = 0.f, sz = 0.f;
-    const float *r = rows + l;
-    for (uint32_t k = 0; k < ns; ++k, r += a.n_total) {
-        sx = sx + r[0];
-        sy = sy + r[plane];
-        if (!planar) sz = sz + r[2 * plane];
-    }
-    float4 p = a.pos_in[l];
-    float4 v = a.vel[l];
-    integrate(p, v, sx * a.G, sy * a.G, sz * a.G, a.dt);
-    a.vel[l] = v;
-    a.pos_out[l] = p;
+    const bool live = l < a.count;
+    float4 p = make_float4(0.f, 0.f, 0.f, 0.f);
+    if (live) {
+        const bool planar = (flags[kBcFlagWordNonPlanar] != generation) && !a.force_3d;
+        const size_t plane = (size_t)ns * a.n_total;
+        float sx = 0.f, sy = 0.f, sz = 0.f;
+        const float *r = rows + l;
+        for (uint32_t k = 0; k < ns; ++k, r += a.n_total) {
+            sx = sx + r[0];
+            sy = sy + r[plane];
+            if (!planar) sz = sz + r[2 * plane];
+        }
+        p = a.pos_in[l];
+        float4 v = a.vel[l];
+        integrate(p, v, sx * a.G, sy * a.G, sz * a.G, a.dt);
+        a.vel[l] = v;
+        a.pos_out[l] = p;
+    }
+    next_planes_store(a.next, live, l, p.x, p.y, p.z);
 }
 
 __global__ __launch_bounds__(256) void pairs_accumulate_kernel(const uint32_t *__restrict__ flags, uint32_t generation, uint32_t force_3d,
@@ -372,14 +376,18 @@
                                                            const float *__restrict__ acc)
 {
     const uint32_t l = blockIdx.x * 256u + threadIdx.x;
-    if (l >= a.count) return;
-    const bool planar = (flags[kBcFlagWordNonPlanar] != generation) && !a.force_3d;
-    const float sx = acc[l], sy = acc[a.n_total + l], sz = planar ? 0.f : acc[2 * (size_t)a.n_total + l];
-    float4 p = a.pos_in[l];
-    float4 v = a.vel[l];
-    integrate(p, v, sx * a.G, sy * a.G, sz * a.G, a.dt);
-    a.vel[l] = v;
-    a.pos_out[l] = p;
+    const bool live = l < a.count;
+    float4 p = make_float4(0.f, 0.f, 0.f, 0.f);
+    if (live) {
+        const bool planar = (flags[kBcFlagWordNonPlanar] != generation) && !a.force_3d;
+        const float sx = acc[l], sy = acc[a.n_total + l], sz = planar ? 0.f : acc[2 * (size_t)a.n_total + l];
+        p = a.pos_in[l];
+        float4 v = a.vel[l];
+        integrate(p, v, sx * a.G, sy * a.G, sz * a.G, a.dt);
+        a.vel[l] = v;
+        a.pos_out[l] = p;
+    }
+    next_planes_store(a.next, live, l, p.x, p.y, p.z);
 }
 
 constexpr uint32_t kPrOneTileMax = 262144u;
diff --git a/nenbody_amd/csrc/nb_selftest.inc b/nenbody_amd/csrc/nb_selftest.inc
--- a/nenbody_amd/csrc/nb_selftest.inc
+++ b/nenbody_amd/csrc/nb_selftest.inc
@@ -356,6 +356,7 @@
             if (rc == NB_OK && e == hipSuccess) {
                 nbk::StepArgs a = step_args(p, pl, n, 0, n, c->pos[c->cur].p, c->pos[c->cur ^ 1].p, c->vel.p, c->scratch.p);
                 a.stamps = stamps;
+                c->chain.invalidate();
                 e = launch_planned(pl, a, c->scratch.p, nullptr, c->stream);
             }
             if (rc == NB_OK && e == hipSuccess) e = hipEventRecord(e1, c->stream);
diff --git a/nenbody_amd/dist.py b/nenbody_amd/dist.py
--- a/nenbody_amd/dist.py
+++ b/nenbody_amd/dist.py
@@ -42,11 +42,19 @@
         with torch.cuda.device(anchor.device) if scope else contextlib.nullcontext():
             check(call(stream))
 
-    def step(self, params, n_total, first, count, pos_in, pos_out, vel, scratch) -> None:
+    def step(self, params, n_total, first, count, pos_in, pos_out, vel, scratch, untouched=None) -> None:
         sp = scratch.data_ptr() if scratch is not None and scratch.numel() else None
         sb = scratch.numel() if scratch is not None else 0
-        self._launch(pos_in, lambda stream: self.lib.nb_launch_step(
-            ctypes.byref(params), n_total, first, count, pos_in.data_ptr(), pos_out.data_ptr(), vel.data_ptr(), sp, sb, stream))
+        if untouched is None:
+            self._launch(pos_in, lambda stream: self.lib.nb_launch_step(
+                ctypes.byref(params), n_total, first, count, pos_in.data_ptr(), pos_out.data_ptr(), vel.data_ptr(), sp, sb, stream))
+        else:
+            self._launch(pos_in, lambda stream: self.lib.nb_chain_step(
+                ctypes.byref(params), n_total, first, count, pos_in.data_ptr(), pos_out.data_ptr(), vel.data_ptr(), sp, sb,
+                _lib.NB_STEP_CHAINED if untouched else 0, stream))
+
+    def scratch_bytes_chained(self, params: NbParams, n_total: int, count: int) -> int:
+        return int(self.lib.nb_chain_bytes(ctypes.byref(params), n_total, count))
 
     def scratch_bytes_phased(self, params: NbParams, n_total: int, count: int, j_lo: int, j_hi: int) -> int:
         return int(self.lib.nb_scratch_bytes_phased(ctypes.byref(params), n_total, count, j_lo, j_hi))
@@ -163,6 +171,7 @@
         self.overlap = bool(overlap) and self.params.mode == _lib.NB_MODE_FAST and world > 1 and not self.partners
         self._pending = None
         self._own_ready = None
+        self.chained = world == 1 and hasattr(self.backend, "scratch_bytes_chained")
         can = bool(self.partners) and hasattr(self.backend, "ring_phased") and self.backend.ring_phased(self.params, self.n, self.first, self.count)
         if ring_overlap and not can:
             raise ValueError("ring_overlap=True: this shape does not run its step in phases (nb_ring_phased() == 0)")
@@ -171,6 +180,8 @@
             sb = self.backend.ring_scratch_bytes(self.params, self.n, self.first, self.count)
         elif self.overlap:
             sb = self.backend.scratch_bytes_phased(self.params, self.n, self.count, self.first, self.first + self.count) if self.count else 0
+        elif self.chained:
+            sb = self.backend.scratch_bytes_chained(self.params, self.n, self.count) if self.count else 0
         else:
             sb = self.backend.scratch_bytes(self.params, self.n, self.count) if self.count else 0
         self.scratch = torch.empty((sb,), dtype=torch.uint8, device=self.device) if sb else None
@@ -488,7 +499,10 @@
             self._pending = self._all_gather_slots(dst, async_op=True)
         else:
             self._wait_pending()
-            if self.count:
+            if self.count and self.chained and self.scratch is not None:
+                self.backend.step(self.params, self.n, self.first, self.count, src, dst, self.vel, self.scratch, untouched=ready)
+                self._own_ready = self.scratch
+            elif self.count:
                 self.backend.step(self.params, self.n, self.first, self.count, src, dst, self.vel, self.scratch)
             if self.world > 1:
                 self._all_gather_slots(dst)
```

Result: no change. 23.55 million (median of 6 runs) (+0.3%).
